# zenlc2000/pycuda-euler

Hardware: AMD Instinct MI355X
Metric: k-mers/sec (encode+hash+deBruijn+Euler), 10Mx100bp k=31, 1/2/4/8 GPU (higher is better)
Workload: dtype u64

## Files before the change

pycuda-euler_amd/csrc/assemble.hip:

```cpp
#include "common.h"
#include "count_global.h"
#include "graph.h"

#include <rocprim/rocprim.hpp>

#include <algorithm>
#include <cmath>
#include <climits>
#include <cstring>
#include <cstddef>
#include <functional>
#include <type_traits>
#include <vector>

#include "count_part.h"
#include "count_v2.h"
#include "count_sk2.h"
#include "shard.h"
#include "compact.h"
#include "count_wide.h"
#include "hostin.h"
#include "join_w.h"
#include "extended.h"
#include "rank_tile.h"
#include "junction.h"
#include "join_local.h"
#include "clip.h"
#include "pop.h"
#include "spectrum.h"
#include "dense_filter.h"

#include <atomic>
#include <chrono>
#include <dlfcn.h>
#include <cstdio>
#include <cstdlib>
#include <mutex>
#include <thread>

namespace ec {

std::atomic<unsigned long long> g_hbm_held{0}, g_hbm_peak{0};
inline void hbm_account(long long d) {
    const unsigned long long now = g_hbm_held.fetch_add((unsigned long long)d) + (unsigned long long)d;
    unsigned long long pk = g_hbm_peak.load();
    while (now > pk && !g_hbm_peak.compare_exchange_weak(pk, now)) {
    }
}
bool memlog_on();

struct DevBuf {
    void *p = nullptr;
    size_t cap = 0;
    __attribute__((noinline)) int ensure(size_t bytes, unsigned int spare_div = 0) {
        if (bytes <= cap) return EC_OK;
        size_t want = std::max<size_t>(bytes, 256);
        if (cap) want += want / 8;
        else if (spare_div) want += want / spare_div;
        release();
        const auto t0 = std::chrono::steady_clock::now();
        if (hipMalloc(&p, want) != hipSuccess) {
            p = nullptr;
            set_error("hipMalloc(%zu) failed", want);
            return EC_ERR_NOMEM;
        }
        cap = want;
        hbm_account((long long)want);
        if (want >= (1ull << 30) && memlog_on()) {
            Dl_info di{};
            void *ra = __builtin_return_address(0);
            const unsigned long off = dladdr(ra, &di) && di.dli_fbase ? (unsigned long)((char *)ra - (char *)di.dli_fbase) : 0ul;
            const double ms = std::chrono::duration<double, std::milli>(std::chrono::steady_clock::now() - t0).count();
            fprintf(stderr, "[eulerhip mem] +%.2f GB (held %.2f GB) in %.1f ms at lib+0x%lx\n", want / 1e9,
                    g_hbm_held.load() / 1e9, ms, off);
        }
        return EC_OK;
    }
    template <typename T>
    T *as() const { return reinterpret_cast<T *>(p); }
    void release() {
        if (p) {
            const auto t0 = std::chrono::steady_clock::now();
            hipFree(p);
            hbm_account(-(long long)cap);
            if (cap >= (1ull << 30) && memlog_on())
                fprintf(stderr, "[eulerhip mem] -%.2f GB (held %.2f GB) in %.1f ms\n", cap / 1e9, g_hbm_held.load() / 1e9,
                        std::chrono::duration<double, std::milli>(std::chrono::steady_clock::now() - t0).count());
        }
        p = nullptr;
        cap = 0;
    }
};

struct HostBuf {
    char *p = nullptr;
    size_t cap = 0, size = 0;
    int resize(size_t bytes) {
        size = bytes;
        if (bytes <= cap) return EC_OK;
        if (p) (void)hipHostFree(p);
        p = nullptr;
        cap = 0;
        size_t want = std::max<size_t>(bytes + bytes / 4, 4096);
        if (hipHostMalloc(reinterpret_cast<void **>(&p), want, hipHostMallocDefault) != hipSuccess) {
            p = nullptr;
            size = 0;
            set_error("hipHostMalloc(%zu) failed", want);
            return EC_ERR_NOMEM;
        }
        cap = want;
        return EC_OK;
    }
    char *data() const { return p; }
    bool empty() const { return size == 0; }
    void release() {
        if (p) (void)hipHostFree(p);
        p = nullptr;
        cap = size = 0;
    }
};

template <typename T>
struct PinnedVec {
    HostBuf b;
    size_t n = 0;
    int resize(size_t count) {
        n = count;
        return b.resize(count * sizeof(T));
    }
    T *data() const { return reinterpret_cast<T *>(b.p); }
    size_t size() const { return n; }
    bool empty() const { return n == 0; }
    T &operator[](size_t i) const { return data()[i]; }
    void release() {
        b.release();
        n = 0;
    }
};

}

using namespace ec;

struct ec_session {
    int device = 0;
    hipStream_t stream = nullptr;
    bool own_stream = false;
    DevBuf h_reads, h_offsets;
    DevBuf hll, scal, table, dkey, dcnt, dfc, dft, upal, outdeg, cand, succ, pred, st0, st1;
    DevBuf rid, rlist, nextR, PK, RK, PL, PM;
    DevBuf hist, ftot, cnt, offs, bstart, tot, recs, recs2, sub;
    DevBuf startOf, skeys, svals, skeys2, svals2, cidxOf, clen, coff, chars, cfirst, clast, headOf, tailOf;
    DevBuf lk, lcnt, tmp, dchars, dcounts;
    bool have = false;
    int k = 0;
    ec_stats stats{};
    HostBuf h_chars;
    bool chars_packed = false;
    uint64_t nchars_host = 0;
    HostBuf bounce;
    struct Pend {
        void *dst;
        size_t off, n;
    };
    std::vector<Pend> pend;
    size_t bused = 0;
    hipEvent_t rd_ev = nullptr;
    hipStream_t ostream = nullptr;
    hipEvent_t oev[4] = {nullptr, nullptr, nullptr, nullptr};
    uint64_t last_nchars = 0;
    DevBuf bmark, rt_tb;
    bool bmark_ok = false;
    uint64_t seg_marks = 0;
    struct SkSpec {
        bool valid = false;
        uint64_t G = 0, cap = 0, nreads = 0, read_base = 0, fcap = 0;
        uint32_t M = 0;
        int k = 0, bbits = 0;
    } skspec;
    struct JlSpec {
        bool valid = false, queued = false;
        int bits = 0, k = 0;
        unsigned int ucap = 0, fcap = 0;
    } jlspec;
    DevBuf jl_frec;
    bool graph_follows = false;
    uint64_t spec_cnt[4] = {0, 0, 0, 0};
    PinnedVec<uint64_t> h_coff;
    PinnedVec<uint64_t> h_loff;
    PinnedVec<int64_t> h_links;
    PinnedVec<uint8_t> h_lc8;
    PinnedVec<uint32_t> h_links32;
    bool links_compact = false;
    HostBuf h_blk;
    bool want_dict = false;
    hipEvent_t ev[2 * EC_NSTAGES] = {};
    hipEvent_t kev[2 * EC_NKERNELS] = {};
    bool kused[EC_NKERNELS] = {};
    bool sused[EC_NSTAGES] = {};
    bool events = false;
    bool timing = false;
    bool stage_timing = false;
    unsigned int n_dense = 0;
    bool dense_ok = false;
    bool stats_ok = false;
    unsigned flags = 0;
    DevBuf ocnt, rbc, mbid, mbid2, midx, midx2, gcur, cwalk, ewalk, lc8;
    bool no_index = false;
    uint64_t shard_base = 0;
    const uint64_t *lc_off = nullptr;
    uint64_t lc_n = 0, lc_L = 0;
    DevBuf bnp;
    DevBuf fcur, bb2;
    DevBuf nrec;
    SolidIndex gidx{};
    SolidIndexW gidxw{};
    bool graph_loaded = false;
    bool placed = false;
    uint64_t seg_lo = 0, seg_Ur = 0;
    DevBuf jrec, joid, jout, jseg, jcnt;
    DevBuf xrec;
    DevBuf skm_rec, skm_ev, skm_end;
    DevBuf wcodes_tab;
    HostBuf hmeta;
    int owner_rule = 0;
    bool own_valid = false;
    int own_rule = 0, own_nowners = 0;
    unsigned int own_n = 0, own_nblk = 0;
    std::vector<unsigned int> own_hi;
    hipStream_t cstream = nullptr;
    struct Pipe {
        bool active = false;
        bool packed = false;
        int nchunks = 0, done = 0;
        std::vector<uint64_t> blo, bhi;
        std::vector<uint64_t> ravail;
        std::vector<uint64_t> elo, ehi;
        uint64_t first_len = 0;
        const uint32_t *codes = nullptr;
        const uint64_t *exc_pos = nullptr;
        const uint8_t *exc_byte = nullptr;
        uint8_t *ascii = nullptr;
        std::vector<hipEvent_t> ev;
    } pipe;
    DevBuf p_codes, p_exc;
    struct Staged {
        Pipe pipe;
        DevBuf codes, exc, off;
        hipEvent_t free_ev = nullptr;
        uint64_t nreads = 0, nbases = 0;
    } stg[2];
    int stg_head = 0, stg_n = 0;
    bool xalpha = false;
    XAlpha xa{};
    DevBuf x_par, x_irr, x_in, x_succ, x_done, x_lk, x_lv, x_lk2, x_lv2, x_len, x_m, x_cid, x_head, x_tail;
    DevBuf jl_kof, jl_rs, jl_re, jl_cnt, jl_off, jl_flag;
    DevBuf rpack;
    DevBuf rt_tcnt, rt_tbase, rt_srec, rt_snrec, rt_sidx, rt_pks, rt_rks, rt_hasp, rt_lr;
    int spec_rounds = 0;
    DevBuf wbv;
    uint64_t seg_n0 = 0, seg_n1 = 0;
    struct Pending {
        int kind = 0;
        uint64_t n = 0;
        unsigned int ntiles = 0;
        bool planned = false;
    } hold;
    SuperRec *chain_scr = nullptr;
    unsigned int seg_nc = 0;
    uint64_t seg_nchars = 0;
    DevBuf run_cnt, run_ends, run_dends;
    DevBuf rt_lb;
    unsigned long long lb_epoch = 0;
    uint64_t run_nr = 0, run_nch = 0, run_nends = 0;
    bool runs_ready = false;
    int part_stage = 0;
    bool clip_ok = false;
    const char *clip_why = "a new session holds no assembly";
    SolidIndex cidx{};
    SolidIndexW cidxw{};
    DevBuf clip_cand, clip_list, clip_kill, clip_tot;
    DevBuf pop_key, pop_sum, pop_tcnt, pop_toff, pop_tile;
    DevBuf spec_hist;
};

static const char *const CLIP_WHY_STEPWISE =
    "the last calls were stepwise ones (ec_count_shard / ec_merge_owned* / ec_graph_*), which leave no one-GPU assembly";

static inline void drop_step_state(ec_session *s) {
    s->hold.kind = 0;
    s->runs_ready = false;
    s->chain_scr = nullptr;
    s->part_stage = 0;
}

namespace {
constexpr size_t BOUNCE_CAP = 64 << 10, BOUNCE_MAX = 16 << 10;

int d2h(ec_session *s, void *dst, const void *src, size_t n, hipStream_t st) {
    if (!n) return EC_OK;
    const size_t off = (s->bused + 15) & ~size_t(15);
    if (n > BOUNCE_MAX || off + n > BOUNCE_CAP) {
        EC_HIP(hipMemcpyAsync(dst, src, n, hipMemcpyDeviceToHost, st));
        return EC_OK;
    }
    if (!s->bounce.p) EC_CHECK(s->bounce.resize(BOUNCE_CAP));
    EC_HIP(hipMemcpyAsync(s->bounce.p + off, src, n, hipMemcpyDeviceToHost, st));
    s->pend.push_back({dst, off, n});
    s->bused = off + n;
    return EC_OK;
}

int host_wait(ec_session *s, hipEvent_t ev) {
    const hipError_t e = hipEventSynchronize(ev);
    for (const auto &q : s->pend) std::memcpy(q.dst, s->bounce.p + q.off, q.n);
    s->pend.clear();
    s->bused = 0;
    if (e != hipSuccess) {
        set_error("HIP error %s", hipGetErrorString(e));
        return EC_ERR_HIP;
    }
    return EC_OK;
}

int host_sync(ec_session *s, hipStream_t st) {
    const hipError_t e = hipStreamSynchronize(st);
    for (const auto &q : s->pend) std::memcpy(q.dst, s->bounce.p + q.off, q.n);
    s->pend.clear();
    s->bused = 0;
    if (e != hipSuccess) {
        set_error("HIP error %s", hipGetErrorString(e));
        return EC_ERR_HIP;
    }
    return EC_OK;
}
}

namespace ec {

template <typename Ops>
__global__ void __launch_bounds__(256) k_kmers_to_agg(const char *chars, const unsigned int *counts, uint64_t n, int k,
                                                      typename RecOf<typename Ops::K>::T *out, unsigned long long *bad) {
    using K = typename Ops::K;
    const K mask = Ops::mask(k);
    for (uint64_t t = blockIdx.x * (uint64_t)blockDim.x + threadIdx.x; t < n; t += (uint64_t)gridDim.x * blockDim.x) {
        const char *x = chars + t * (uint64_t)k;
        K code{};
        bool ok = true;
        for (int i = 0; i < k; i++) {
            const uint32_t b = base_code((unsigned char)x[i]);
            ok &= b < 4;
            code = Ops::push(code, b & 3u, mask);
        }
        if (!ok) atomicMin(bad, (unsigned long long)t);
        const K tw = Ops::twin(code, k);
        out[t] = RecOf<K>::make(code < tw ? code : tw, code <= tw ? counts[t] : 0u,
                                code <= tw ? (unsigned long long)t : ~0ull, tw <= code ? (unsigned long long)t : ~0ull);
    }
}
}

namespace {

struct Scalars {
    unsigned long long npos;
    unsigned long long bad;
    unsigned long long ndistinct;
    double est;
    unsigned int overflow;
    unsigned int nsolid;
    unsigned int nstarts;
    unsigned int final_sel;
    unsigned int ndict;
    unsigned int nr;
    unsigned int npal;
    unsigned int ngath;
    unsigned long long nvisited;
    unsigned int maxlocal;
    unsigned int skew;
    unsigned int lens[4];
    unsigned long long nrec;
    unsigned int nasym, nxl, nxs;
    unsigned int xbad;
    unsigned int wbv_long, wpad;
    unsigned long long chains;
    unsigned int active[64];
};
static_assert(sizeof(Scalars) % 8 == 0 && offsetof(Scalars, bad) % 8 == 0, "k_scal_reset writes 64-bit words");

__global__ void __launch_bounds__(64) k_scal_reset(Scalars *sc) {
    unsigned long long *w = reinterpret_cast<unsigned long long *>(sc);
    for (unsigned int i = threadIdx.x; i < sizeof(Scalars) / 8; i += 64)
        w[i] = i == offsetof(Scalars, bad) / 8 ? ~0ull : 0ull;
}

__global__ void __launch_bounds__(256) k_emit_init(unsigned int *a, unsigned int *b, unsigned int *c, uint64_t n,
                                                   unsigned int *flag) {
    const uint64_t t0 = blockIdx.x * (uint64_t)blockDim.x + threadIdx.x, st = (uint64_t)gridDim.x * blockDim.x;
    if (t0 == 0) *flag = 0;
    const uint64_t n4 = n / 4;
    const uint4 v = make_uint4(0xFFFFFFFFu, 0xFFFFFFFFu, 0xFFFFFFFFu, 0xFFFFFFFFu);
    uint4 *a4 = reinterpret_cast<uint4 *>(a), *b4 = reinterpret_cast<uint4 *>(b), *c4 = reinterpret_cast<uint4 *>(c);
    for (uint64_t i = t0; i < n4; i += st) {
        a4[i] = v;
        b4[i] = v;
        c4[i] = v;
    }
    for (uint64_t i = 4 * n4 + t0; i < n; i += st) a[i] = b[i] = c[i] = 0xFFFFFFFFu;
}

int scan_u64(ec_session *s, const unsigned long long *in, unsigned long long *out, size_t n) {
    size_t bytes = 0;
    EC_HIP(rocprim::exclusive_scan(nullptr, bytes, in, out, 0ull, n, rocprim::plus<unsigned long long>(), s->stream));
    EC_CHECK(s->tmp.ensure(bytes));
    EC_HIP(rocprim::exclusive_scan(s->tmp.p, bytes, in, out, 0ull, n, rocprim::plus<unsigned long long>(), s->stream));
    return EC_OK;
}

int scan_excl_u32(ec_session *s, const unsigned int *in, unsigned int *out, size_t n) {
    size_t bytes = 0;
    EC_HIP(rocprim::exclusive_scan(nullptr, bytes, in, out, 0u, n, rocprim::plus<unsigned int>(), s->stream));
    EC_CHECK(s->tmp.ensure(bytes));
    EC_HIP(rocprim::exclusive_scan(s->tmp.p, bytes, in, out, 0u, n, rocprim::plus<unsigned int>(), s->stream));
    return EC_OK;
}

int scan_incl_u32(ec_session *s, const unsigned int *in, unsigned int *out, size_t n) {
    size_t bytes = 0;
    EC_HIP(rocprim::inclusive_scan(nullptr, bytes, in, out, n, rocprim::plus<unsigned int>(), s->stream));
    EC_CHECK(s->tmp.ensure(bytes));
    EC_HIP(rocprim::inclusive_scan(s->tmp.p, bytes, in, out, n, rocprim::plus<unsigned int>(), s->stream));
    return EC_OK;
}

int sort_pairs(ec_session *s, unsigned long long *kin, unsigned long long *kout, unsigned int *vin, unsigned int *vout,
               size_t n) {
    size_t bytes = 0;
    EC_HIP(rocprim::radix_sort_pairs(nullptr, bytes, kin, kout, vin, vout, n, 0, 64, s->stream));
    EC_CHECK(s->tmp.ensure(bytes));
    EC_HIP(rocprim::radix_sort_pairs(s->tmp.p, bytes, kin, kout, vin, vout, n, 0, 64, s->stream));
    return EC_OK;
}

int pipe_upto(ec_session *s, int c) {
    auto &pp = s->pipe;
    if (!pp.active) return EC_OK;
    c = std::min(c, pp.nchunks - 1);
    if (pp.done > c) return EC_OK;
    const int first = pp.done;
    for (; pp.done <= c; pp.done++) EC_HIP(hipStreamWaitEvent(s->stream, pp.ev[pp.done], 0));
    const uint64_t blo = pp.blo[first], bhi = pp.bhi[c], elo = pp.elo[first], ehi = pp.ehi[c];
    if (pp.packed && bhi > blo) {
        const uint64_t units = ((bhi + 15) >> 4) - (blo >> 4);
        k_unpack2<<<grid_for(units, 256, 16384), 256, 0, s->stream>>>(pp.codes, blo, bhi, pp.ascii);
        if (ehi > elo)
            k_patch<<<grid_for(ehi - elo, 256, 4096), 256, 0, s->stream>>>(pp.exc_pos, pp.exc_byte, elo, ehi,
                                                                           pp.ascii);
    }
    return EC_OK;
}
int pipe_all(ec_session *s) { return s->pipe.active ? pipe_upto(s, s->pipe.nchunks - 1) : EC_OK; }

inline void mark(ec_session *s, int idx) {
    if (s->stage_timing) {
        hipEventRecord(s->ev[idx], s->stream);
        if (idx & 1) s->sused[idx >> 1] = true;
    }
}
inline void kmark(ec_session *s, int kid, int end) {
    if (s->timing) {
        hipEventRecord(s->kev[2 * kid + end], s->stream);
        if (end) s->kused[kid] = true;
    }
}

void collect_timing(ec_session *s) {
    if (!s->timing) return;
    hipStreamSynchronize(s->stream);
    for (int i = 0; i < EC_NSTAGES; i++) {
        float ms = 0;
        if (s->stage_timing && s->sused[i]) hipEventElapsedTime(&ms, s->ev[2 * i], s->ev[2 * i + 1]);
        s->stats.stage_ms[i] = ms;
    }
    for (int i = 0; i < EC_NKERNELS; i++) {
        float ms = 0;
        if (s->kused[i]) hipEventElapsedTime(&ms, s->kev[2 * i], s->kev[2 * i + 1]);
        s->stats.kernel_ms[i] = ms;
    }
}

int begin_call(ec_session *s, int k, unsigned flags) {
    s->xalpha = false;
    drop_step_state(s);
    s->graph_loaded = false;
    s->dense_ok = false;
    s->clip_ok = false;
    s->clip_why = "the session's last call failed";
    refresh_knobs();
    s->have = false;
    s->stats_ok = false;
    if (k < 1 || k > EC_MAX_K) {
        set_error("k=%d outside [1,%d]", k, EC_MAX_K);
        return EC_ERR_ARG;
    }
    EC_HIP(hipSetDevice(s->device));
    if (s->ostream) EC_HIP(hipStreamSynchronize(s->ostream));
    memset(&s->stats, 0, sizeof(s->stats));
    s->k = k;
    s->want_dict = (flags & EC_FLAG_WANT_DICT) != 0;
    s->flags = flags;
    s->shard_base = 0;
    s->own_valid = false;
    s->bmark_ok = false;
    s->seg_marks = 0;
    s->placed = false;
    const bool timing = (flags & (EC_FLAG_TIMING | EC_FLAG_KERNEL_TIMING)) != 0;
    s->stage_timing = (flags & EC_FLAG_TIMING) != 0;
    if (timing && !s->events) {
        for (auto &e : s->ev) EC_HIP(hipEventCreate(&e));
        for (auto &e : s->kev) EC_HIP(hipEventCreate(&e));
        s->events = true;
    }
    s->timing = timing;
    for (auto &u : s->kused) u = false;
    for (auto &u : s->sused) u = false;
    EC_CHECK(s->scal.ensure(sizeof(Scalars)));
    s->jlspec.queued = false;
    s->graph_follows = false;
    k_scal_reset<<<1, 64, 0, s->stream>>>(s->scal.as<Scalars>());
    return EC_OK;
}


template <typename SlotT, typename KeyT>
int compact_table(ec_session *s, SlotT *table, uint64_t cap, long long limit, KeyT *dkey) {
    hipStream_t st = s->stream;
    Scalars *dsc = s->scal.as<Scalars>();
    const unsigned int nblk = (unsigned int)((cap + COMPACT_CHUNK - 1) / COMPACT_CHUNK);
    EC_CHECK(s->rbc.ensure((size_t)nblk * 8 + 8));
    unsigned int *bc = s->rbc.as<unsigned int>(), *bs = bc + nblk;
    EC_HIP(hipMemsetAsync(&dsc->nsolid, 0, 4, st));
    EC_HIP(hipMemsetAsync(&dsc->ndistinct, 0, 8, st));
    k_compact_count<SlotT><<<nblk, 256, 0, st>>>(table, cap, limit, bc, &dsc->ndistinct);
    EC_CHECK(scan_incl_u32(s, bc, bs, nblk));
    k_compact_write<SlotT, KeyT><<<nblk, 256, 0, st>>>(table, cap, limit, bs, dkey, s->dcnt.as<unsigned int>(),
                                                      s->dfc.as<unsigned long long>(),
                                                      s->dft.as<unsigned long long>());
    k_compact_total<<<1, 1, 0, st>>>(bs, nblk, &dsc->nsolid);
    return EC_OK;
}


int check_node_ids(unsigned int U) {
    if (2ull * U >= (unsigned long long)CYC) {
        set_error("too many solid k-mers (%u) for 31-bit node ids", U);
        return EC_ERR_CAPACITY;
    }
    return EC_OK;
}

int check_alphabet(const uint8_t *d_reads, unsigned long long bad) {
    if (bad == ~0ull) return EC_OK;
    uint8_t byte = 0;
    hipMemcpy(&byte, d_reads + bad, 1, hipMemcpyDeviceToHost);
    set_error("byte %llu (0x%02x) outside {A,C,G,T,N}", bad, byte);
    return EC_ERR_ALPHABET;
}

struct BucketArgs {
    const unsigned long long *bbeg = nullptr, *bend = nullptr;
    bool filt = false;
    int pmin = 0, pmax = 1;
    unsigned int *bmark = nullptr;
};
BucketArgs filter_args(bool filt, int pmax) {
    BucketArgs a;
    a.filt = filt;
    a.pmax = pmax;
    a.pmin = kn().filter_pmin >= 0 ? std::max(0, std::min(pmax, kn().filter_pmin)) : 0;
    return a;
}

template <typename Src>
int launch_bucket(ec_session *s, Src src, unsigned nb, unsigned slots, long long limit, BucketArgs a = {}) {
    Scalars *dsc = s->scal.as<Scalars>();
    hipStream_t st = s->stream;
    const unsigned long long *bb = a.bbeg ? a.bbeg : s->bstart.as<unsigned long long>();
    const unsigned long long *be = a.bbeg ? a.bend : s->bstart.as<unsigned long long>() + 1;
    if (a.filt) {
        EC_CHECK(s->bnp.ensure(nb));
        k_bucket_filt<Src><<<nb, BUCKET_THREADS, 0, st>>>(
            src, bb, be, 1u, limit, a.pmin, a.pmax, (float)PART_KEYS,
            s->dkey.as<unsigned long long>(),
            s->dcnt.as<unsigned int>(), s->dfc.as<unsigned long long>(), s->dft.as<unsigned long long>(),
            s->no_index ? nullptr : s->sub.as<SubSlot>(), s->bnp.as<uint8_t>(), &dsc->nsolid, &dsc->ndistinct,
            &dsc->overflow);
        return EC_OK;
    }
    if (slots == 2048)
        k_bucket<Src, 2048><<<nb, BUCKET_THREADS, 0, st>>>(
            src, bb, be, 1u, limit, s->dkey.as<unsigned long long>(), s->dcnt.as<unsigned int>(),
            s->dfc.as<unsigned long long>(), s->dft.as<unsigned long long>(), s->no_index ? nullptr : s->sub.as<SubSlot>(), &dsc->nsolid,
            &dsc->ndistinct, &dsc->overflow, a.bmark);
    else
        k_bucket<Src, 4096><<<nb, BUCKET_THREADS, 0, st>>>(
            src, bb, be, 1u, limit, s->dkey.as<unsigned long long>(), s->dcnt.as<unsigned int>(),
            s->dfc.as<unsigned long long>(), s->dft.as<unsigned long long>(), s->no_index ? nullptr : s->sub.as<SubSlot>(), &dsc->nsolid,
            &dsc->ndistinct, &dsc->overflow, a.bmark);
    return EC_OK;
}

struct BucketPlan {
    bool part = false;
    bool filt = false;
    int pmax = 1;
    int bbits = 0;
    unsigned int slots = 2048;
};
BucketPlan plan_buckets(double est, long long limit) {
    constexpr int PMAX = 3;
    BucketPlan p;
    const double filt_max = limit >= 1 ? 32768.0 : PART_KEYS * (1 << PMAX);
    p.part = est / FINE <= 2400.0 || est / FINE <= filt_max;
    p.filt = p.part && (est / FINE > 2400.0 || kn().force_filter);
    while (p.pmax < PMAX && est / FINE / (double)(1 << p.pmax) > PART_KEYS) p.pmax++;
    if (kn().filter_pmax) p.pmax = std::max(1, std::min(PMAX, kn().filter_pmax));
    while (p.bbits < FINE_BITS && est / (double)(1ull << p.bbits) > 1100.0) p.bbits++;
    p.slots = p.filt ? (2048u << p.pmax) : est / (double)(1ull << p.bbits) > 1100.0 ? 4096u : 2048u;
    return p;
}

static uint64_t skpart_slots(int npf, int w, bool val) {
    static thread_local int cache[3][SK_W_MAX + 1][2] = {};
    const int ni = npf == 4 ? 0 : npf == 7 ? 1 : 2;
    int &c = cache[ni][w][val];
    if (!c) {
        const void *fn = nullptr;
#define EC_SKF(NPF, W)                                                                                        \
    if (npf == NPF && w == W) fn = val ? (const void *)&k_skpart_w<NPF, W, true> : (const void *)&k_skpart_w<NPF, W, false>;
#define EC_SKF_W(W) EC_SKF(4, W) EC_SKF(7, W) EC_SKF(10, W)
        EC_SKF_W(7) EC_SKF_W(8) EC_SKF_W(9) EC_SKF_W(10) EC_SKF_W(11) EC_SKF_W(12)
        EC_SKF_W(13) EC_SKF_W(14) EC_SKF_W(15) EC_SKF_W(16) EC_SKF_W(17) EC_SKF_W(18)
#undef EC_SKF_W
#undef EC_SKF
        int dev = 0, ncu = 0, per = 0;
        if (!fn || hipGetDevice(&dev) != hipSuccess ||
            hipDeviceGetAttribute(&ncu, hipDeviceAttributeMultiprocessorCount, dev) != hipSuccess ||
            hipOccupancyMaxActiveBlocksPerMultiprocessor(&per, fn, PT_THREADS, 0) != hipSuccess || per < 1)
            return 1;
        c = ncu * per;
    }
    return (uint64_t)c;
}

int phase_count_sk2(ec_session *s, const uint8_t *d_reads, const uint64_t *d_off, uint64_t nreads,
                    uint64_t read_base, int k, long long limit, uint32_t M, uint64_t G, uint64_t gsize, uint64_t P,
                    int npf, unsigned int &U, SolidIndex &sidx, bool &done, bool validate = false,
                    bool *invalid = nullptr) {
    done = false;
    if (invalid) *invalid = false;
    if (k >= SK_MIN_K && k <= 32) {
        const uint64_t ntiles = (nreads + 63) / 64, slots = skpart_slots(npf, k - SK_M + 1, validate);
        uint64_t g = std::max<uint64_t>(1, std::min<uint64_t>(ntiles, RF_MAX_RUNS));
        if (g > slots) g = g / slots * slots;
        gsize = ((ntiles + g - 1) / g) * 64;
        G = (nreads + gsize - 1) / gsize;
    }
    if (k < SK_MIN_K || k > 32 || M > 256 || gsize * M >= (1ull << 24) || (read_base + nreads) * 2 * M >= (1ull << 32) ||
        kn().no_sk2)
        return EC_OK;
    hipStream_t st = s->stream;
    Scalars *dsc = s->scal.as<Scalars>();
    Scalars hsc;
    auto reset = [&]() -> int {
        if (validate) {
            EC_HIP(hipMemsetAsync(dsc, 0, sizeof(Scalars), st));
            EC_HIP(hipMemsetAsync(&dsc->bad, 0xFF, sizeof(unsigned long long), st));
            return EC_OK;
        }
        EC_HIP(hipMemsetAsync(&dsc->overflow, 0, sizeof(unsigned int), st));
        EC_HIP(hipMemsetAsync(&dsc->skew, 0, sizeof(unsigned int), st));
        EC_HIP(hipMemsetAsync(&dsc->nsolid, 0, sizeof(unsigned int), st));
        EC_HIP(hipMemsetAsync(&dsc->ndistinct, 0, sizeof(unsigned long long), st));
        return EC_OK;
    };
    const MinCfg mc = sk_cfg(k);
    constexpr uint64_t C = 1ull << SK2_CBITS;
    const double per_read = 2.0 * M / (mc.w + 1) + 2.0;
    const uint64_t cap = (uint64_t)(gsize * per_read * 1.4 / C) + 256;
    EC_CHECK(s->recs.ensure((C * G * cap + SK2_ECAP_W) * 16));
    EC_CHECK(s->cnt.ensure(C * G * 4));
    EC_CHECK(s->hll.ensure(G * (1 << HLL_REG_BITS)));
    EC_CHECK(s->ftot.ensure((1 << HLL_REG_BITS) * 4));
    uint4 *recs = s->recs.as<uint4>();
    const uint32_t smask = P >= (1ull << 26) ? 255u : 0u;
    unsigned int *hreg = s->ftot.as<unsigned int>();
    if (!validate) EC_HIP(hipMemsetAsync(&dsc->nrec, 0, sizeof(unsigned long long), st));
    mark(s, 2 * EC_STAGE_COUNT);
    kmark(s, 1, 0);
#define EC_SKPART_WV(NPF, W, VAL)                                                                             \
    k_skpart_w<NPF, W, VAL><<<lgb - lga, PT_THREADS, 0, st>>>(                                                   \
        d_reads, d_off, nreads, mc, M, gsize, (uint32_t)G, cap, smask, recs, s->cnt.as<unsigned int>(),          \
        s->hll.as<uint8_t>(), &dsc->nrec, &dsc->overflow, &dsc->lens[2], &dsc->npos, lga, elim)
#define EC_SKPART_W(NPF, W)            \
    if (validate)                      \
        EC_SKPART_WV(NPF, W, true);    \
    else                               \
        EC_SKPART_WV(NPF, W, false)
#define EC_SKPART_NPF(W)              \
    if (npf == 4) EC_SKPART_W(4, W);  \
    else if (npf == 7) EC_SKPART_W(7, W); \
    else EC_SKPART_W(10, W)
    const bool chunked = s->pipe.active && s->pipe.done < s->pipe.nchunks;
    if (!chunked) EC_CHECK(pipe_all(s));
    unsigned lga = 0, lgb = (unsigned)G;
    const uint32_t elim = kn().sk2_elim >= 128 ? (uint32_t)std::min(kn().sk2_elim, SK2_ECAP_W) : (uint32_t)SK2_ECAP_W;
    for (int pc = chunked ? 0 : s->pipe.nchunks; ; pc++) {
      if (chunked) {
        if (pc >= s->pipe.nchunks) break;
        lgb = pc + 1 == s->pipe.nchunks ? (unsigned)G : (unsigned)std::min<uint64_t>(G, s->pipe.ravail[pc] / gsize);
        if (lgb <= lga) continue;
        EC_CHECK(pipe_upto(s, pc));
      }
      {
        switch (mc.w) {
            case 7: EC_SKPART_NPF(7); break;
            case 8: EC_SKPART_NPF(8); break;
            case 9: EC_SKPART_NPF(9); break;
            case 10: EC_SKPART_NPF(10); break;
            case 11: EC_SKPART_NPF(11); break;
            case 12: EC_SKPART_NPF(12); break;
            case 13: EC_SKPART_NPF(13); break;
            case 14: EC_SKPART_NPF(14); break;
            case 15: EC_SKPART_NPF(15); break;
            case 16: EC_SKPART_NPF(16); break;
            case 17: EC_SKPART_NPF(17); break;
            default: EC_SKPART_NPF(18); break;
        }
      }
      if (!chunked) break;
      lga = lgb;
    }
#undef EC_SKPART_NPF
#undef EC_SKPART_W
#undef EC_SKPART_WV
    kmark(s, 1, 1);
    EC_HIP(hipMemsetAsync(hreg, 0, (1 << HLL_REG_BITS) * 4, st));
    k_hll_merge<<<dim3((1 << HLL_REG_BITS) / 256, TOT_SLICES), 256, 0, st>>>(s->hll.as<uint8_t>(), G, hreg);
    k_hll_final<<<1, 1024, 0, st>>>(hreg, HLL_REG_BITS, &dsc->est);
    EC_CHECK(d2h(s, &hsc, dsc, sizeof(Scalars), st));
    auto launch_refine = [&](int bb, uint64_t fc) -> int {
        const uint64_t nb = 1ull << bb;
        EC_CHECK(s->recs2.ensure(nb * fc * 16));
        EC_CHECK(s->fcur.ensure(nb * 8));
        EC_CHECK(s->bb2.ensure(nb * 16));
        EC_HIP(hipMemsetAsync(s->fcur.p, 0, nb * 8, st));
        unsigned rs = 8;
        if (kn().refine_rs) rs = (unsigned)std::max(1, kn().refine_rs);
        rs = (unsigned)std::min<uint64_t>(rs, G);
        kmark(s, 4, 0);
        k_skrefine<<<dim3((unsigned)C, rs), BUCKET_THREADS, 0, st>>>(recs, s->cnt.as<unsigned int>(), (uint32_t)G, cap,
                                                                      bb, s->recs2.as<uint4>(), fc,
                                                                      s->fcur.as<unsigned long long>(), &dsc->skew, M,
                                                                      gsize, read_base, k);
        kmark(s, 4, 1);
        unsigned long long *b0 = s->bb2.as<unsigned long long>();
        k_fixed_bounds<<<grid_for(nb, 256), 256, 0, st>>>(s->fcur.as<unsigned long long>(), nb, fc, b0, b0 + nb);
        return EC_OK;
    };
    const auto sp = s->skspec;
    const bool spec = sp.valid && sp.G == G && sp.cap == cap && sp.nreads == nreads && sp.read_base == read_base &&
                      sp.M == M && sp.k == k && !chunked && kn().no_spec == 0;
    s->skspec.valid = false;
    if (spec) {
        if (!s->rd_ev) EC_HIP(hipEventCreateWithFlags(&s->rd_ev, hipEventDisableTiming));
        EC_HIP(hipEventRecord(s->rd_ev, st));
        EC_CHECK(launch_refine(sp.bbits, sp.fcap));
        EC_CHECK(host_wait(s, s->rd_ev));
    } else {
        EC_CHECK(host_sync(s, st));
    }
    const bool verbose = kn().verbose;
    if (validate) {
        if (hsc.lens[2]) {
            if (verbose) fprintf(stderr, "count_sk2: input needs the prescan\n");
            if (invalid) *invalid = true;
            return reset();
        }
        P = hsc.npos;
    }
    if (hsc.overflow) {
        if (verbose) fprintf(stderr, "count_sk2: partition run overflow (cap %llu)\n", (unsigned long long)cap);
        return reset();
    }
    const double est = hsc.est * (smask + 1.0);
    BucketPlan plan = plan_buckets(est, limit);
    const bool skfilt = plan.part && plan.filt && limit >= 1 && kn().sk_filt != 0 &&
                        est / (double)(1ull << SK2_BBITS) <= 16000.0;
    if (!plan.part || (plan.filt && !skfilt)) return reset();
    int bbits = SK2_CBITS;
    const bool b3 = !skfilt && !kn().no_skb3 && est / (double)(1ull << SK2_BBITS) <= 380.0;
    const double per_bucket = b3 ? 380.0 : 800.0;
    while (bbits < SK2_BBITS && est / (double)(1ull << bbits) > per_bucket) bbits++;
    if (skfilt) bbits = SK2_BBITS;
    plan.bbits = bbits;
    plan.slots = skfilt ? 2048u : b3 ? 1024u : est / (double)(1ull << bbits) > 1100.0 ? 4096u : 2048u;
    const uint64_t Bk = 1ull << bbits;
    const uint64_t NR = hsc.nrec;
    uint64_t fcap = NR * 2 / Bk + 1024;
    const bool refine_stood = spec && sp.bbits == bbits && sp.fcap >= fcap && sp.fcap <= fcap + fcap / 8;
    if (refine_stood) {
        fcap = sp.fcap;
    } else {
        if (spec && verbose) fprintf(stderr, "count_sk2: refine plan changed (bits %d -> %d), refined again\n", sp.bbits, bbits);
        fcap += fcap / 16;
        EC_CHECK(launch_refine(bbits, fcap));
    }
    s->skspec.valid = true;
    s->skspec.G = G;
    s->skspec.cap = cap;
    s->skspec.nreads = nreads;
    s->skspec.read_base = read_base;
    s->skspec.fcap = fcap;
    s->skspec.M = M;
    s->skspec.k = k;
    s->skspec.bbits = bbits;
    unsigned long long *bbeg = s->bb2.as<unsigned long long>(), *bend = bbeg + Bk;
    mark(s, 2 * EC_STAGE_COUNT + 1);

    mark(s, 2 * EC_STAGE_COMPACT);
    const uint64_t umax = Bk * plan.slots;
    EC_CHECK(s->dkey.ensure(umax * 8));
    EC_CHECK(s->dcnt.ensure(umax * 4));
    EC_CHECK(s->dfc.ensure(umax * 8));
    EC_CHECK(s->dft.ensure(umax * 8));
    EC_CHECK(s->sub.ensure(umax * sizeof(SubSlot)));
    bool b3_marked = false;
    for (int attempt = 0;; attempt++) {
    kmark(s, 2, 0);
    const double inv_m = 1.0 / M;
#define EC_SKBUCKET_ARGS                                                                                     \
    s->recs2.as<uint4>(), bbeg, bend, k, M, inv_m, limit, s->dkey.as<unsigned long long>(),                    \
        s->dcnt.as<unsigned int>(), s->dfc.as<unsigned long long>(), s->dft.as<unsigned long long>(),          \
        s->no_index ? nullptr : s->sub.as<SubSlot>(), &dsc->nsolid, &dsc->ndistinct, &dsc->overflow
#define EC_SKBUCKET(SLOTS, RS, EVEN) \
    k_skbucket<SLOTS, RS, 1, EVEN><<<(unsigned)Bk, BUCKET_THREADS, 0, st>>>(EC_SKBUCKET_ARGS, dbg)
    b3_marked = false;
    unsigned long long *dbg = nullptr;
    if (kn().sk2_stats) {
        EC_CHECK(s->tmp.ensure(128));
        dbg = s->tmp.as<unsigned long long>();
        EC_HIP(hipMemsetAsync(dbg, 0, 128, st));
    }
    if (skfilt) {
        constexpr int NTF = 512;
        const unsigned int max_keys = kn().skf_keys > 0 ? (unsigned int)kn().skf_keys : 1900u;
        unsigned int *bm = nullptr;
        if (kn().skf_merge != 0) {
            EC_CHECK(s->skm_rec.ensure(Bk * fcap * sizeof(uint4)));
            EC_CHECK(s->skm_ev.ensure(Bk * fcap * sizeof(uint2)));
            EC_CHECK(s->skm_end.ensure(Bk * 8));
            uint4 *mrec = s->skm_rec.as<uint4>();
            uint2 *mev = s->skm_ev.as<uint2>();
            unsigned long long *mend = s->skm_end.as<unsigned long long>();
            const unsigned int claim_cap = kn().sk2_claim > 0 ? (unsigned int)kn().sk2_claim : ~0u;
            if (kn().skf_merge != 2)
                k_skdedup<4096, 1024><<<(unsigned)Bk, 1024, 0, st>>>(s->recs2.as<uint4>(), bbeg, bend, k, M, inv_m, mrec,
                                                                     mev, mend, claim_cap, dbg);
            else
                k_skdedup<2560, 512><<<(unsigned)Bk, 512, 0, st>>>(s->recs2.as<uint4>(), bbeg, bend, k, M, inv_m, mrec,
                                                                   mev, mend, claim_cap, dbg);
#define EC_SKF_MERGED_ARGS                                                                                   \
    mrec, bbeg, mend, k, M, inv_m, limit, s->dkey.as<unsigned long long>(), s->dcnt.as<unsigned int>(),      \
        s->dfc.as<unsigned long long>(), s->dft.as<unsigned long long>(),                                    \
        s->no_index ? nullptr : s->sub.as<SubSlot>(), &dsc->nsolid, &dsc->ndistinct, &dsc->overflow, max_keys, \
        dbg, bm, mev
            if (k & 1)
                k_skbucket_filt<2048, NTF, false, true><<<(unsigned)Bk, NTF, 0, st>>>(EC_SKF_MERGED_ARGS);
            else
                k_skbucket_filt<2048, NTF, true, true><<<(unsigned)Bk, NTF, 0, st>>>(EC_SKF_MERGED_ARGS);
#undef EC_SKF_MERGED_ARGS
        } else if (k & 1)
            k_skbucket_filt<2048, NTF, false><<<(unsigned)Bk, NTF, 0, st>>>(EC_SKBUCKET_ARGS, max_keys, dbg, bm);
        else
            k_skbucket_filt<2048, NTF, true><<<(unsigned)Bk, NTF, 0, st>>>(EC_SKBUCKET_ARGS, max_keys, dbg, bm);
        b3_marked = bm != nullptr;
    } else if (plan.slots == 1024) {
        constexpr int NT3 = 512;
        const unsigned int claim_cap = kn().sk2_claim > 0 ? (unsigned int)kn().sk2_claim : ~0u;
        const size_t words = (umax / 32 + 2 + 63) & ~size_t(63);
        EC_CHECK(s->bmark.ensure(words * 4));
        EC_HIP(hipMemsetAsync(s->bmark.p, 0, words * 4, st));
        unsigned int *bm = s->bmark.as<unsigned int>();
        if (dbg) {
            if (k & 1)
                k_skbucket3<1024, 1664, NT3, false, true><<<(unsigned)Bk, NT3, 0, st>>>(EC_SKBUCKET_ARGS, dbg, claim_cap, bm);
            else
                k_skbucket3<1024, 1664, NT3, true, true><<<(unsigned)Bk, NT3, 0, st>>>(EC_SKBUCKET_ARGS, dbg, claim_cap, bm);
        } else if (k & 1)
            k_skbucket3<1024, 1664, NT3, false><<<(unsigned)Bk, NT3, 0, st>>>(EC_SKBUCKET_ARGS, dbg, claim_cap, bm);
        else
            k_skbucket3<1024, 1664, NT3, true><<<(unsigned)Bk, NT3, 0, st>>>(EC_SKBUCKET_ARGS, dbg, claim_cap, bm);
        b3_marked = true;
    } else if (plan.slots == 2048) {
        if (k & 1) EC_SKBUCKET(2048, 3072, false);
        else EC_SKBUCKET(2048, 3072, true);
    } else {
        if (k & 1) EC_SKBUCKET(4096, 2048, false);
        else EC_SKBUCKET(4096, 2048, true);
    }
#undef EC_SKBUCKET
#undef EC_SKBUCKET_ARGS
    if (dbg) {
        unsigned long long h[16];
        EC_CHECK(d2h(s, h, dbg, 128, st));
        EC_CHECK(host_sync(s, st));
        const double nw = (double)Bk * ((plan.slots == 1024 ? 512 : BUCKET_THREADS) / 64);
        if (skfilt)
            fprintf(stderr, "k_skbucket_filt: %llu buckets: max distinct est %llu, max predicted inserts %llu, max "
                            "seen-twice cells %llu, max records %llu; refused by the predictor %llu, tables filled "
                            "%llu, most keys inserted %llu; most merged records %llu, most past the claim cap %llu, "
                            "merged records %llu of %llu\n",
                    (unsigned long long)Bk, h[0], h[1], h[2], h[3], h[4], h[5], h[6], h[7], h[8], h[9],
                    (unsigned long long)NR);
        if (plan.slots == 1024)
            fprintf(stderr, "k_skbucket3: %llu buckets, most distinct records in a bucket %llu\n",
                    (unsigned long long)Bk, h[3]);
        fprintf(stderr, "k_skbucket per wave (shader clocks): records phase canon %.0f probe %.0f (%.1f iterations) "
                        "post %.0f barrier %.0f over %.1f rounds; roll-out %.0f barrier %.0f\n",
                h[8] / nw, h[9] / nw, h[11] / nw, h[10] / nw, h[12] / nw, h[13] / nw, h[14] / nw, h[15] / nw);
        fprintf(stderr, "k_skbucket: %llu records, %llu distinct in %llu flushes (%.2f / bucket), %llu windows rolled "
                        "(positions %llu); block-us: init %.0f records %.0f sort %.0f roll-out %.0f finish %.0f\n",
                (unsigned long long)NR, h[0], h[1], (double)h[1] / Bk, h[2], (unsigned long long)P, h[3] / 100.0,
                h[4] / 100.0, h[5] / 100.0, h[6] / 100.0, h[7] / 100.0);
    }
    kmark(s, 2, 1);
    mark(s, 2 * EC_STAGE_COMPACT + 1);
    EC_CHECK(d2h(s, &hsc, dsc, sizeof(Scalars), st));
    const auto jp = s->jlspec;
    s->jlspec.queued = false;
    if (!attempt && refine_stood && jp.valid && s->graph_follows && !s->no_index && !skfilt && !dbg &&
        (k & 1) && jp.k == k && jp.bits == bbits && kn().jl_bits_delta == 0 && kn().jl_fcap <= 0 &&
        kn().join_links != 0 && kn().join_local != 0) {
        const unsigned int ntab = 1u << jp.bits;
        EC_CHECK(s->jl_kof.ensure((size_t)jp.ucap * 4));
        EC_CHECK(s->jl_rs.ensure((size_t)ntab * 4));
        EC_CHECK(s->jl_re.ensure((size_t)ntab * 4));
        EC_CHECK(s->jl_cnt.ensure(((size_t)ntab + 1) * 4));
        EC_CHECK(s->jl_off.ensure(((size_t)ntab + 1) * 4));
        EC_CHECK(s->jl_flag.ensure((size_t)(JL_NCTR + 1) * JL_CSTRIDE * 4));
        EC_CHECK(s->jl_frec.ensure((size_t)jp.fcap * sizeof(RecJ64)));
        EC_CHECK(s->upal.ensure(jp.ucap));
        EC_CHECK(s->succ.ensure((size_t)jp.ucap * 8));
        if (!s->rd_ev) EC_HIP(hipEventCreateWithFlags(&s->rd_ev, hipEventDisableTiming));
        EC_HIP(hipEventRecord(s->rd_ev, st));
        unsigned int *flags = s->jl_flag.as<unsigned int>();
        k_jl_init<<<grid_for(2ull * jp.ucap, 256, 4096), 256, 0, st>>>(
            flags, (JL_NCTR + 1) * JL_CSTRIDE, s->jl_rs.as<unsigned int>(), s->jl_cnt.as<unsigned int>(), ntab,
            s->succ.as<unsigned int>(), 2ull * jp.ucap, s->upal.as<uint8_t>(), jp.ucap);
        k_jl_scan<unsigned long long><<<grid_for(jp.ucap, 256, 8192), 256, 0, st>>>(
            s->dkey.as<unsigned long long>(), jp.ucap, k, jp.bits, s->upal.as<uint8_t>(), s->jl_kof.as<unsigned int>(),
            s->jl_frec.as<RecJ64>(), flags + JL_CSTRIDE, jp.fcap, s->jl_cnt.as<unsigned int>(),
            s->jl_rs.as<unsigned int>(), s->jl_re.as<unsigned int>(), &flags[1], &dsc->nsolid, &flags[2]);
        EC_CHECK(host_wait(s, s->rd_ev));
        s->jlspec.queued = true;
        if (hsc.skew || hsc.overflow || hsc.nsolid > jp.ucap) {
            s->jlspec.queued = false;
            s->spec_cnt[1]++;
        }
    } else {
        EC_CHECK(host_sync(s, st));
    }
    if (!hsc.skew || attempt) break;
    std::vector<unsigned long long> hcur(Bk);
    EC_CHECK(d2h(s, hcur.data(), s->fcur.p, Bk * 8, st));
    EC_CHECK(host_sync(s, st));
    const uint64_t need = *std::max_element(hcur.begin(), hcur.end());
    if (need <= fcap || need > 4 * fcap || Bk * need * 16 > (1ull << 30)) break;
    if (verbose)
        fprintf(stderr, "count_sk2: final bucket overflow (fcap %llu), refined again with capacity %llu\n",
                (unsigned long long)fcap, (unsigned long long)need);
    fcap = need;
    EC_HIP(hipMemsetAsync(&dsc->overflow, 0, sizeof(unsigned int), st));
    EC_HIP(hipMemsetAsync(&dsc->skew, 0, sizeof(unsigned int), st));
    EC_HIP(hipMemsetAsync(&dsc->nsolid, 0, sizeof(unsigned int), st));
    EC_HIP(hipMemsetAsync(&dsc->ndistinct, 0, sizeof(unsigned long long), st));
    EC_CHECK(launch_refine(bbits, fcap));
    }
    if (hsc.overflow || hsc.skew) {
        if (verbose)
            fprintf(stderr, "count_sk2: %s overflow (%llu buckets, %u slots, est %.0f, fcap %llu)\n",
                    hsc.skew ? "final bucket" : "table", (unsigned long long)Bk, plan.slots, est,
                    (unsigned long long)fcap);
        s->stats.table_retries++;
        return reset();
    }
    done = true;
    s->bmark_ok = b3_marked;
    s->stats.n_positions = P;
    s->stats.n_distinct_est = (uint64_t)llround(est);
    s->stats.record_bytes = 16;
    s->stats.n_records = NR;
    s->stats.count_path = EC_PATH_PARTITIONED;
    s->stats.count_variant = 3;
    s->stats.n_buckets = (uint32_t)Bk;
    s->stats.table_capacity = umax;
    sidx = SolidIndex{};
    sidx.sub = s->sub.as<SubSlot>();
    sidx.bbits = bbits;
    sidx.slots = plan.slots;
    sidx.sk = 1;
    sidx.mc = mc;
    sidx.npb = nullptr;
    U = hsc.nsolid;
    s->stats.n_distinct = hsc.ndistinct;
    s->stats.n_solid = U;
    return check_node_ids(U);
}

int phase_count_v2(ec_session *s, const uint8_t *d_reads, const uint64_t *d_off, uint64_t nreads, uint64_t read_base,
                   int k, long long limit, bool allow_sk2, unsigned int &U, SolidIndex &sidx, bool &ok) {
    ok = false;
    hipStream_t st = s->stream;
    Scalars *dsc = s->scal.as<Scalars>();
    Scalars hsc;
    const uint64_t ntiles = (nreads + 63) / 64;
    uint64_t gmax = RF_MAX_RUNS;
    uint64_t G = std::max<uint64_t>(1, std::min<uint64_t>(ntiles, gmax));
    const uint64_t gsize = ((ntiles + G - 1) / G) * 64;
    G = (nreads + gsize - 1) / gsize;
    auto npf_of = [](uint64_t lall) {
        const uint64_t need16 = (64ull * lall + 30 + 15) / 16;
        return need16 <= 4 * 64 ? 4 : need16 <= 7 * 64 ? 7 : need16 <= 10 * 64 ? 10 : 0;
    };
    if (allow_sk2 && k >= SK_MIN_K && k <= 32 && !kn().no_sk2) {
        uint64_t L = s->lc_L;
        if (s->pipe.active) {
            L = s->pipe.first_len;
        } else if (!(L >= (uint64_t)k && npf_of(L) && s->lc_off == d_off && s->lc_n == nreads)) {
            uint64_t o2[2] = {0, 0};
            EC_CHECK(d2h(s, o2, d_off, 16, st));
            EC_CHECK(host_sync(s, st));
            L = o2[1] - o2[0];
        }
        s->lc_L = 0;
        const int npf = npf_of(L);
        if (L >= (uint64_t)k && npf) {
            const uint32_t M = (uint32_t)(L - k + 1);
            bool done = false, invalid = false;
            mark(s, 2 * EC_STAGE_PRESCAN);
            mark(s, 2 * EC_STAGE_PRESCAN + 1);
            EC_CHECK(phase_count_sk2(s, d_reads, d_off, nreads, read_base, k, limit, M, G, gsize, nreads * M, npf, U,
                                     sidx, done, true, &invalid));
            if (done) {
                if (!s->pipe.active) s->lc_off = d_off, s->lc_n = nreads, s->lc_L = L;
                ok = true;
                return EC_OK;
            }
            if (!invalid) allow_sk2 = false;
        }
    }
    EC_CHECK(pipe_all(s));
    mark(s, 2 * EC_STAGE_PRESCAN);
    kmark(s, 0, 0);
    k_prescan<<<(unsigned)G, 256, 0, st>>>(d_reads, d_off, nreads, k, gsize, &dsc->npos, &dsc->bad, dsc->lens);
    kmark(s, 0, 1);
    mark(s, 2 * EC_STAGE_PRESCAN + 1);
    EC_CHECK(d2h(s, &hsc, dsc, sizeof(Scalars), st));
    EC_CHECK(host_sync(s, st));
    EC_CHECK(check_alphabet(d_reads, hsc.bad));
    const unsigned int lmax = hsc.lens[0], lmin = ~hsc.lens[1], lall = hsc.lens[3];
    const uint64_t P = hsc.npos;
    if (hsc.lens[2] || P == 0 || lmax != lmin) return EC_OK;
    const uint32_t M = lmax - (uint32_t)k + 1;
    int ibits = 1;
    while ((1ull << ibits) < M) ibits++;
    if (ibits > 15 || nreads + read_base > (1ull << (31 - ibits)) || 2ull * M - 1 > MAX_LOCAL_EVENT) return EC_OK;
    const int npf = npf_of(lall);
    if (!npf) return EC_OK;
    if (allow_sk2) {
        bool done = false;
        EC_CHECK(phase_count_sk2(s, d_reads, d_off, nreads, read_base, k, limit, M, G, gsize, P, npf, U, sidx, done));
        if (done) {
            ok = true;
            return EC_OK;
        }
    }

    auto nbits = [](uint64_t x) {
        int b = 0;
        while ((1ull << b) < x) b++;
        return b;
    };
    const int r10env = kn().v2_r10;
    const bool r10 = r10env != 0 && (r10env == 1 || P >= (1ull << 26)) && k >= 16 &&
                     (2 * k - PT_CBITS) + std::max(0, nbits(gsize) + 1 + ibits - 16) <= 64;

    constexpr uint64_t C = 1ull << PT_CBITS;
    const uint64_t cap = (gsize * M * 5 / 4 + C - 1) / C + 128;
    EC_CHECK(s->recs.ensure((C * G * cap + PT_REC) * 12));
    EC_CHECK(s->cnt.ensure(C * G * 4));
    EC_CHECK(s->hll.ensure(G * (1 << HLL_REG_BITS)));
    EC_CHECK(s->ftot.ensure((1 << HLL_REG_BITS) * 4));
    unsigned long long *rkeys = s->recs.as<unsigned long long>();
    unsigned int *rmeta = reinterpret_cast<unsigned int *>(rkeys + C * G * cap + PT_REC);
    const uint32_t smask = P >= (1ull << 26) ? 255u : 0u;
    unsigned int *hreg = s->ftot.as<unsigned int>();
    mark(s, 2 * EC_STAGE_COUNT);
    kmark(s, 1, 0);
#define EC_PARTITION(NPF, HI, R10)                                                                            \
    k_partition<NPF, HI, R10><<<(unsigned)G, PT_THREADS, 0, st>>>(d_reads, d_off, nreads, k, M, gsize, (uint32_t)G, \
                                                                   cap, ibits, read_base, smask, rkeys, rmeta,        \
                                                                   s->cnt.as<unsigned int>(),                         \
                                                                   s->hll.as<uint8_t>(), &dsc->overflow)
#define EC_PARTITION_R(NPF, HI)        \
    if (r10)                           \
        EC_PARTITION(NPF, HI, true);   \
    else                               \
        EC_PARTITION(NPF, HI, false)
    if (k >= 17) {
        if (npf == 4) EC_PARTITION_R(4, true);
        else if (npf == 7) EC_PARTITION_R(7, true);
        else EC_PARTITION_R(10, true);
    } else {
        if (npf == 4) EC_PARTITION_R(4, false);
        else if (npf == 7) EC_PARTITION_R(7, false);
        else EC_PARTITION_R(10, false);
    }
#undef EC_PARTITION_R
#undef EC_PARTITION
    kmark(s, 1, 1);
    EC_HIP(hipMemsetAsync(hreg, 0, (1 << HLL_REG_BITS) * 4, st));
    k_hll_merge<<<dim3((1 << HLL_REG_BITS) / 256, TOT_SLICES), 256, 0, st>>>(s->hll.as<uint8_t>(), G, hreg);
    k_hll_final<<<1, 1024, 0, st>>>(hreg, HLL_REG_BITS, &dsc->est);
    EC_CHECK(d2h(s, &hsc, dsc, sizeof(Scalars), st));
    EC_CHECK(host_sync(s, st));
    if (hsc.overflow) return EC_OK;
    const double est = hsc.est * (smask + 1.0);
    BucketPlan plan = plan_buckets(est, limit);
    if (!plan.part) return EC_OK;
    plan.bbits = std::max(plan.bbits, PT_CBITS);
    const int bbits = plan.bbits;
    const uint64_t Bk = 1ull << bbits;

    const uint64_t fcap = P * 5 / 4 / Bk + 1024;
    EC_CHECK(s->recs2.ensure(Bk * fcap * 12));
    EC_CHECK(s->fcur.ensure(Bk * 8));
    EC_CHECK(s->bb2.ensure(Bk * 16));
    EC_HIP(hipMemsetAsync(s->fcur.p, 0, Bk * 8, st));
    unsigned rs = 8;
    if (kn().refine_rs) rs = (unsigned)std::max(1, kn().refine_rs);
    rs = (unsigned)std::min<uint64_t>(rs, G);
    kmark(s, 4, 0);
#define EC_REFINE(IN10)                                                                                           \
    k_refine2<IN10><<<dim3((unsigned)C, rs), BUCKET_THREADS, 0, st>>>(                                          \
        rkeys, rmeta, s->cnt.as<unsigned int>(), (uint32_t)G, cap, bbits, s->recs2.as<unsigned int>(), fcap,     \
        s->fcur.as<unsigned long long>(), &dsc->skew, k, ibits, gsize, read_base)
    if (r10)
        EC_REFINE(true);
    else
        EC_REFINE(false);
#undef EC_REFINE
    kmark(s, 4, 1);
    unsigned long long *bbeg = s->bb2.as<unsigned long long>(), *bend = bbeg + Bk;
    k_fixed_bounds<<<grid_for(Bk, 256), 256, 0, st>>>(s->fcur.as<unsigned long long>(), Bk, fcap, bbeg, bend);
    mark(s, 2 * EC_STAGE_COUNT + 1);

    mark(s, 2 * EC_STAGE_COMPACT);
    const uint64_t umax = Bk * plan.slots;
    EC_CHECK(s->dkey.ensure(umax * 8));
    EC_CHECK(s->dcnt.ensure(umax * 4));
    EC_CHECK(s->dfc.ensure(umax * 8));
    EC_CHECK(s->dft.ensure(umax * 8));
    EC_CHECK(s->sub.ensure(umax * sizeof(SubSlot)));
    BucketArgs ba = filter_args(plan.filt, plan.pmax);
    ba.bbeg = bbeg;
// ... 4180 lines not shown
```

pycuda-euler_amd/csrc/capi.cpp:

```cpp
#include <cstdarg>
#include <cstdio>
#include <cstdlib>

#include "common.h"

namespace ec {
static thread_local char g_err[512] = "";

void set_error(const char *fmt, ...) {
    va_list ap;
    va_start(ap, fmt);
    vsnprintf(g_err, sizeof g_err, fmt, ap);
    va_end(ap);
}

static thread_local Knobs g_knobs;
const Knobs &kn() { return g_knobs; }
void refresh_knobs() {
    Knobs k;
    if (getenv("EULERHIP_DEBUG")) {
        auto flag = [](const char *n) { return getenv(n) != nullptr; };
        auto num = [](const char *n, int dflt) {
            const char *e = getenv(n);
            return e ? atoi(e) : dflt;
        };
        k.no_sk2 = flag("EULERHIP_NO_SK2");
        k.force_filter = flag("EULERHIP_FORCE_FILTER");
        k.filter_pmax = num("EULERHIP_FILTER_PMAX", 0);
        k.filter_pmin = num("EULERHIP_FILTER_PMIN", -1);
        k.v2_r10 = num("EULERHIP_V2_R10", -1);
        k.refine_rs = num("EULERHIP_REFINE_RS", 0);
        k.no_spec = num("EULERHIP_NO_SPEC", 0);
        k.rank_sync = num("EULERHIP_RANK_SYNC", 0);
        k.skf_merge = num("EULERHIP_SKF_MERGE", 1);
        k.wide_runs = num("EULERHIP_WIDE_RUNS", 1);
        k.no_small_starts = flag("EULERHIP_NO_SMALL_STARTS");
        k.wide_max_bbits = num("EULERHIP_WIDE_MAX_BBITS", -1);
        k.wide_l3 = num("EULERHIP_WIDE_L3", 0);
        k.join_links = num("EULERHIP_JOIN_LINKS", -1);
        k.join_cap = num("EULERHIP_JOIN_CAP", 0);
        k.junction_bt = num("EULERHIP_JUNCTION_BT", -1);
        k.sk2_elim = num("EULERHIP_SK2_ELIM", 0);
        k.no_char_pack = num("EULERHIP_NO_CHAR_PACK", 0);
        k.junction_sb = num("EULERHIP_JUNCTION_SB", 0);
        k.junction_claim = num("EULERHIP_JUNCTION_CLAIM", 0);
        if (const char *e = getenv("EULERHIP_WIDE_L3_CAP")) k.wide_l3_cap = atoll(e);
        k.host_chunks = num("EULERHIP_HOST_CHUNKS", 0);
        k.sk2_stats = flag("EULERHIP_SK2_STATS");
        k.no_skb3 = flag("EULERHIP_NO_SKB3");
        k.sk2_claim = num("EULERHIP_SK2_CLAIM", 0);
        k.verbose = flag("EULERHIP_VERBOSE");
        k.rank = num("EULERHIP_RANK", -1);
        k.sk_filt = num("EULERHIP_SK_FILT", -1);
        k.skf_keys = num("EULERHIP_SKF_KEYS", 0);
        k.wide_mb = num("EULERHIP_WIDE_MB", -1);
        k.join_mb = num("EULERHIP_JOIN_MB", -1);
        k.join_local = num("EULERHIP_JOIN_LOCAL", -1);
        k.junction_radix = num("EULERHIP_JUNCTION_RADIX", -1);
        k.jl_fcap = num("EULERHIP_JL_FCAP", -1);
        k.jl_bits_delta = num("EULERHIP_JL_BITS_DELTA", 0);
    }
    g_knobs = k;
}
bool memlog_on() {
    static const bool on = getenv("EULERHIP_MEMLOG") != nullptr;
    return on;
}
}

extern "C" const char *ec_last_error(void) { return ec::g_err; }
extern "C" int ec_version(void) { return 500;  }

extern "C" int ec_spectrum_threshold(const uint64_t *h, uint32_t nbins, ec_spectrum_info *info) {
    if (nbins < 2 || nbins > EC_SPECTRUM_MAX_BINS) {
        ec::set_error("ec_spectrum_threshold: nbins %u outside [2, %d]", nbins, EC_SPECTRUM_MAX_BINS);
        return EC_ERR_ARG;
    }
    if (!h || !info) {
        ec::set_error("ec_spectrum_threshold: null hist / info");
        return EC_ERR_ARG;
    }
    *info = ec_spectrum_info{};
    uint32_t lo = 0;
    while (lo < nbins && !h[lo]) lo++;
    if (lo == nbins) return EC_OK;
    info->lo = lo;
    uint32_t d = lo;
    while (d + 1 < nbins && h[d] >= h[d + 1]) d++;
    if (d + 1 >= nbins) return EC_OK;
    info->descent_end = d;
    if (d == lo) return EC_OK;
    uint32_t p = d;
    for (uint32_t c = d + 1; c < nbins; c++)
        if (h[c] > h[p]) p = c;
    info->peak = p;
    if (p == nbins - 1) return EC_OK;
    uint64_t m = h[lo];
    for (uint32_t c = lo; c <= p; c++) m = h[c] < m ? h[c] : m;
    info->floor = m;
    uint32_t v = lo;
    const uint64_t within = (h[p] - m) / EC_SPECTRUM_FLOOR_DIV;
    while (v < p && h[v] - m > within) v++;
    if (v == p) return EC_OK;
    info->found = 1;
    info->limit = v;
    return EC_OK;
}
```

pycuda-euler_amd/csrc/common.h:

```cpp
#pragma once
#include <cstring>
#include <hip/hip_runtime.h>
#include <stdint.h>
#include <stdio.h>
#include <string>

#include "../../include/eulerhip.h"

namespace ec {

constexpr uint32_t NONE32 = 0xFFFFFFFFu;
constexpr uint64_t NONE64 = ~0ull;
constexpr uint64_t EMPTY_KEY = ~0ull;

void set_error(const char *fmt, ...);

struct Knobs {
    bool no_sk2 = false;
    bool force_filter = false;
    int filter_pmax = 0;
    int filter_pmin = -1;
    int v2_r10 = -1;
    int refine_rs = 0;
    int rank_sync = 0;
    int no_spec = 0;
    int skf_merge = 1;
    int wide_runs = 1;
    int wide_max_bbits = -1;
    int wide_l3 = 0;
    long long wide_l3_cap = 0;
    int wide_mb = -1;
    int join_links = -1;
    int join_cap = 0;
    int join_local = -1;
    int join_mb = -1;
    int jl_fcap = -1;
    int jl_bits_delta = 0;
    int junction_bt = -1;
    int junction_sb = 0;
    int junction_claim = 0;
    int junction_radix = -1;
    int no_char_pack = 0;
    int sk2_elim = 0;
    int sk2_claim = 0;
    bool sk2_stats = false;
    bool no_skb3 = false;
    int sk_filt = -1;
    int skf_keys = 0;
    int host_chunks = 0;
    bool verbose = false;
    int rank = -1;
    bool no_small_starts = false;
};
void refresh_knobs();
const Knobs &kn();

#define EC_HIP(call)                                                                       \
    do {                                                                                   \
        hipError_t e_ = (call);                                                            \
        if (e_ != hipSuccess) {                                                            \
            ::ec::set_error("%s:%d %s -> %s", __FILE__, __LINE__, #call, hipGetErrorString(e_)); \
            return EC_ERR_HIP;                                                             \
        }                                                                                  \
    } while (0)

#define EC_CHECK(call)                 \
    do {                               \
        int rc_ = (call);              \
        if (rc_ != EC_OK) return rc_;  \
    } while (0)

__host__ __device__ inline uint64_t kmask64(int k) { return k >= 32 ? ~0ull : ((1ull << (2 * k)) - 1); }

__host__ __device__ inline uint64_t rev2_64(uint64_t x) {
    x = ((x >> 2) & 0x3333333333333333ull) | ((x & 0x3333333333333333ull) << 2);
    x = ((x >> 4) & 0x0F0F0F0F0F0F0F0Full) | ((x & 0x0F0F0F0F0F0F0F0Full) << 4);
#if defined(__HIP_DEVICE_COMPILE__)
    return __builtin_bswap64(x);
#else
    return __builtin_bswap64(x);
#endif
}

__host__ __device__ inline uint64_t twin64(uint64_t x, int k) { return rev2_64(x ^ kmask64(k)) >> (64 - 2 * k); }

__host__ __device__ inline uint64_t mix64(uint64_t x) {
    x ^= x >> 29;
    x *= 0xbf58476d1ce4e5b9ull;
    x ^= x >> 32;
    return x;
}

constexpr uint64_t BIJ_C = 0xbf58476d1ce4e5b9ull;
constexpr uint64_t BIJ_CINV = 0x96de1b173f119089ull;
__host__ __device__ inline uint64_t bij_fwd(uint64_t x, int s, uint64_t m) {
    x ^= x >> s;
    x = (x * BIJ_C) & m;
    return x ^ (x >> s);
}
__host__ __device__ inline uint64_t bij_inv(uint64_t x, int s, uint64_t m) {
    x ^= x >> s;
    x = (x * BIJ_CINV) & m;
    return x ^ (x >> s);
}

__device__ inline uint32_t base_code(uint32_t c) {
    switch (c) {
    case 'A': return 0;
    case 'C': return 1;
    case 'G': return 2;
    case 'T': return 3;
    case 'N': return 4;
    default: return 5;
    }
}

__device__ inline unsigned int wave_append(unsigned int *counter, bool pred) {
    const unsigned long long m = __ballot(pred);
    if (!m) return 0;
    const unsigned int lane = threadIdx.x & 63;
    const int leader = __ffsll((long long)m) - 1;
    unsigned int base = 0;
    if ((int)lane == leader) base = atomicAdd(counter, (unsigned int)__popcll(m));
    base = __shfl(base, leader);
    return base + (unsigned int)__popcll(m & ((1ull << lane) - 1));
}

inline unsigned grid_for(uint64_t n, unsigned block, unsigned cap = 1u << 20) {
    uint64_t g = (n + block - 1) / block;
    if (g < 1) g = 1;
    if (g > cap) g = cap;
    return (unsigned)g;
}

}
```

pycuda-euler_amd/csrc/count_sk2.h:

```cpp
#pragma once
#include "count_v2.h"
#include "superkmer.h"

namespace ec {

constexpr int SK2_NMAX = 16;
constexpr int SK2_ECAP_W = 1024;
constexpr int SK2_FLUSH_AT = SK2_ECAP_W - 64 - 640;
#ifndef SK2_PD_DEF
#define SK2_PD_DEF 4
#endif
constexpr int SK2_PD = SK2_PD_DEF;
constexpr int SK2_HQ = 128;
constexpr int SK2_BASES = 46;
#ifndef SK2_TILE_DEF
#define SK2_TILE_DEF 2048
#endif
constexpr int SK2_TILE = SK2_TILE_DEF;
constexpr int SK2_CBITS = 6;
constexpr int SK2_BBITS = 14;
constexpr int SK2_FBITS = SK2_BBITS - SK2_CBITS;

__host__ __device__ constexpr inline uint32_t sk2_nmax(int k) {
    return (uint32_t)(SK2_BASES - k + 1 < SK2_NMAX ? SK2_BASES - k + 1 : SK2_NMAX);
}

__device__ inline uint32_t sk_bases16(const uint32_t *st, uint32_t p) {
    return __builtin_amdgcn_alignbit(st[(p >> 4) + 1], st[p >> 4], 2 * (p & 15));
}
__device__ inline void sk_hll_put(unsigned int *s_hll, uint32_t hh) {
    const uint32_t hj = hh >> (32 - HLL_REG_BITS);
    const uint32_t rho = (uint32_t)__clz((int)((hh << HLL_REG_BITS) | (1u << (HLL_REG_BITS - 1)))) + 1;
    const uint32_t hs = (hj & 3) * 8;
    uint32_t old = s_hll[hj >> 2];
    while (rho > ((old >> hs) & 0xFFu)) {
        const uint32_t nw = (old & ~(0xFFu << hs)) | (rho << hs);
        const uint32_t prev = atomicCAS(&s_hll[hj >> 2], old, nw);
        if (prev == old) break;
        old = prev;
    }
}

template <int C>
__device__ inline void skpart_flush(uint32_t cntw, const uint32_t *ent, uint16_t *srt, unsigned int *wcnt,
                                    unsigned int *cur, unsigned long long *base, const uint32_t *rel,
                                    const uint32_t *st, uint32_t lane, unsigned long long gcap, uint64_t cap,
                                    unsigned long long spill, uint32_t M, uint32_t rtile, uint4 *recs,
                                    unsigned int *overflow, unsigned int *s_hll, uint32_t *hq, uint32_t smaskb,
                                    int k, uint64_t kmask) {
    wave_sync();
    for (uint32_t i = lane; i < cntw; i += 64) atomicAdd(&wcnt[ent[i] >> 26], 1u);
    wave_sync();
    const unsigned int v = lane < (uint32_t)C ? wcnt[lane] : 0u;
    const unsigned int incl = wave_incl_scan(v);
    const unsigned int beg = incl - v;
    if (lane < (uint32_t)C) {
        wcnt[lane] = beg;
        unsigned int at = 0;
        if (v) at = atomicAdd(&cur[lane], v);
        unsigned long long b0 = gcap + lane * cap + at - beg;
        if (at + v > cap) {
            atomicOr(overflow, 1u);
            b0 = spill - beg;
        }
        base[lane] = b0;
    }
    wave_sync();
    for (uint32_t i = lane; i < cntw; i += 64) {
        const unsigned int p = atomicAdd(&wcnt[ent[i] >> 26], 1u);
        srt[p] = (uint16_t)i;
    }
    wave_sync();
    uint32_t nq = 0;
    auto hll_drain = [&]() {
        wave_sync();
        for (uint32_t x = lane; x < nq * SK2_NMAX; x += 64) {
            const uint32_t qe = hq[x / SK2_NMAX], q = x % SK2_NMAX;
            if (q <= (qe >> 16)) {
                const uint32_t p = (qe & 0xFFFFu) + q;
                const uint64_t K = (uint64_t)sk_bases16(st, p) | (uint64_t)sk_bases16(st, p + 16) << 32;
                const uint64_t krc = ~K & kmask, kfw = rev2_64(K) >> (64 - 2 * k);
                sk_hll_put(s_hll, (uint32_t)(mix64(kfw < krc ? kfw : krc) >> 32));
            }
        }
        wave_sync();
        nq = 0;
    };
    for (uint32_t i0 = 0; i0 < cntw; i0 += 64) {
        const uint32_t i = i0 + lane;
        bool samp = false;
        uint32_t qv = 0;
        if (i < cntw) {
            const uint32_t e = ent[srt[i]];
            const uint32_t lr = e & 63u, w0 = (e >> 6) & 0xFFu, n1 = (e >> 14) & 15u;
            const uint32_t p0 = rel[lr] + w0;
            uint4 o;
            o.x = sk_bases16(st, p0);
            o.y = sk_bases16(st, p0 + 16);
            o.z = (sk_bases16(st, p0 + 32) & 0x0FFFFFFFu) | n1 << 28;
            o.w = ((e >> 18) & ((1u << SK2_FBITS) - 1)) << 24 | ((rtile + lr) * M + w0);
            recs[base[e >> 26] + i] = o;
            samp = ((e >> 18) & smaskb) == 0;
            qv = p0 | n1 << 16;
        }
        const uint64_t sb = __builtin_amdgcn_ballot_w64(samp);
        if (samp) hq[nq + __builtin_amdgcn_mbcnt_hi((uint32_t)(sb >> 32), __builtin_amdgcn_mbcnt_lo((uint32_t)sb, 0u))] = qv;
        nq += (uint32_t)__popcll(sb);
        if (nq > (uint32_t)(SK2_HQ - 64)) hll_drain();
    }
    if (nq) hll_drain();
    wave_sync();
    if (lane < (uint32_t)C) wcnt[lane] = 0;
}

template <int NPF, int W, bool VAL>
__global__ void __launch_bounds__(PT_THREADS) k_skpart_w(const uint8_t *__restrict__ buf,
                                                         const uint64_t *__restrict__ off, uint64_t nreads, MinCfg mc,
                                                         uint32_t M, uint64_t gsize, uint32_t G, uint64_t cap,
                                                         uint32_t smask, uint4 *recs, unsigned int *cnt, uint8_t *hll,
                                                         unsigned long long *nrec, unsigned int *overflow,
                                                         unsigned int *vfail, unsigned long long *npos,
                                                         uint32_t g_lo, uint32_t elim) {
    constexpr int C = 1 << SK2_CBITS;
    constexpr int NREG = 1 << HLL_REG_BITS;
    constexpr int SW = NPF * 64 + 4;
    static_assert(SK2_FLUSH_AT >= 64, "the entry buffer holds a flush's worth");
    __shared__ uint32_t s_stage[PT_WAVES][SW];
    __shared__ uint32_t s_ent[PT_WAVES][SK2_ECAP_W];
    __shared__ uint16_t s_srt[PT_WAVES][SK2_ECAP_W];
    __shared__ uint32_t s_rel[PT_WAVES][64];
    __shared__ unsigned long long s_base[PT_WAVES][C];
    __shared__ unsigned int s_wcnt[PT_WAVES][C];
    __shared__ unsigned int s_cur[C];
    __shared__ unsigned int s_hll[NREG / 4];
    __shared__ uint32_t s_hq[PT_WAVES][SK2_HQ];
    const uint32_t lane = threadIdx.x & 63;
    const uint32_t wid = __builtin_amdgcn_readfirstlane(threadIdx.x >> 6);
    for (int i = threadIdx.x; i < NREG / 4; i += PT_THREADS) s_hll[i] = 0;
    if (threadIdx.x < C) s_cur[threadIdx.x] = 0;
    if (lane < C) s_wcnt[wid][lane] = 0;
    __syncthreads();
    const uint64_t g = blockIdx.x + (uint64_t)g_lo;
    const uint64_t g0 = min(g * gsize, nreads), g1 = min(g0 + gsize, nreads);
    const uint32_t ntile = (uint32_t)((g1 - g0 + 63) / 64);
    const int k = mc.k;
    constexpr uint32_t nmax = sk2_nmax(W + SK_M - 1);
    const uint64_t kmask = kmask64(k);
    uint4 pf[NPF];
    uint64_t nx_base = 0;
    uint32_t nx_s = 0, nx_e = 0, nx_n = 0, nx_lo = 0, nx_hi = 0, nx_n16 = 0;
    uint32_t nwin = 0;
    if (wid < ntile) EC_PT_ISSUE(wid);
    const unsigned long long gcap = g * C * cap, spill = (unsigned long long)C * G * cap;
    uint32_t *st = s_stage[wid];
    uint32_t *ent = s_ent[wid];
    for (uint32_t t = wid; t < ntile; t += PT_WAVES) {
        if (VAL) {
            uint32_t diff = 0;
#pragma unroll
            for (int q = 0; q < NPF; q++) {
                const uint32_t wv[4] = {pf[q].x, pf[q].y, pf[q].z, pf[q].w};
                uint32_t packed = 0, d[4];
#pragma unroll
                for (int u = 0; u < 4; u++) {
                    const uint32_t x = ((wv[u] >> 1) ^ (wv[u] >> 2)) & 0x03030303u;
                    const uint32_t y = x | (x >> 6);
                    packed |= ((y | (y >> 12)) & 0xFFu) << (8 * u);
                    d[u] = __builtin_amdgcn_perm(0u, 0x54474341u, x) ^ wv[u];
                }
                st[q * 64 + lane] = packed;
                const uint32_t lo = 16 * (q * 64 + lane);
                if (lo >= nx_lo && lo + 16 <= nx_hi) {
                    diff |= d[0] | d[1] | d[2] | d[3];
                } else if (lo < nx_hi && lo + 16 > nx_lo) {
                    const uint32_t from = (uint32_t)min(max((int)nx_lo - (int)lo, 0), 16);
                    const uint32_t to = (uint32_t)min(max((int)nx_hi - (int)lo, 0), 16);
                    const uint32_t m16 = (0xFFFFu >> (16 - to)) & ~((1u << from) - 1u);
#pragma unroll
                    for (int u = 0; u < 4; u++) {
                        const uint32_t m4 = (m16 >> (4 * u)) & 15u;
                        const uint32_t keep = ((m4 * 0x00204081u) & 0x01010101u) * 0xFFu;
                        diff |= d[u] & keep;
                    }
                }
            }
            bool bad = nx_n16 > (uint32_t)NPF * 64 || diff != 0;
            if (lane < nx_n) {
                const uint32_t ln = nx_e - nx_s;
                bad |= ln >= (uint32_t)k && ln != M + (uint32_t)k - 1;
            }
            if (__any(bad) && lane == 0) atomicOr(vfail, 1u);
            nwin += (uint32_t)__popcll(__ballot(lane < nx_n && nx_e - nx_s >= (uint32_t)k));
        } else {
#pragma unroll
            for (int q = 0; q < NPF; q++) st[q * 64 + lane] = pack16(pf[q]);
        }
        const uint32_t tbase = (uint32_t)nx_base, s = nx_s;
        const uint32_t len = lane < nx_n ? nx_e - nx_s : 0u;
        const bool more = t + PT_WAVES < ntile;
        const bool has = len >= (uint32_t)k;
        const uint32_t rel = has ? s - tbase : 0u;
        s_rel[wid][lane] = rel;
        wave_sync();
        constexpr int m = SK_M;
        constexpr uint32_t MMASK = (1u << (2 * SK_M)) - 1;
        uint32_t mf = 0, mr = 0;
        auto push_base = [&](uint32_t b) {
            mf = ((mf << 2) | b) & MMASK;
            mr = (mr >> 2) | ((3u - b) << (2 * SK_M - 2));
        };
        uint32_t S[W];
        {
            const uint32_t x0 = sk_bases16(st, rel), x1 = sk_bases16(st, rel + 16);
#pragma unroll
            for (int tb = 0; tb < m - 1; tb++) push_base(tb < 16 ? (x0 >> (2 * tb)) & 3u : (x1 >> (2 * (tb - 16))) & 3u);
#pragma unroll
            for (int j = 0; j < W; j++) {
                const int tb = m - 1 + j;
                push_base(tb < 16 ? (x0 >> (2 * tb)) & 3u : (x1 >> (2 * (tb - 16))) & 3u);
                S[j] = mmer_hash(mf < mr ? mf : mr);
            }
#pragma unroll
            for (int j = W - 2; j >= 0; j--) S[j] = min(S[j], S[j + 1]);
        }
        const uint32_t nrounds = __any(has) ? (M + W - 1) / W : 0u;
        uint32_t runv = S[0], rsx = 0, cntw = 0;
        const uint64_t hasm = __builtin_amdgcn_ballot_w64(has);
        const uint32_t rtile = 64 * t;
        auto entry = [&](uint32_t end) { return (runv << 18) + lane + (((end - 1u) << 14) + rsx); };
        auto rs_term = [](uint32_t w) { return (uint32_t)((int)w * -16320); };
        for (uint32_t round = 0; round < nrounds; round++) {
            const uint32_t w0 = round * W;
            const uint32_t q = rel + w0 + W;
            const uint32_t a0 = sk_bases16(st, q), a1 = sk_bases16(st, q + 16);
            const uint32_t rw0 = rs_term(w0);
            uint32_t H[W];
            uint32_t P = 0xFFFFFFFFu;
            auto window = [&](int j) {
                const uint32_t v = min(S[j], P);
                const int tb = m - 1 + j;
                const uint32_t b = tb < 16 ? (a0 >> (2 * tb)) & 3u : (a1 >> (2 * (tb - 16))) & 3u;
                mf = (mf << 2) | b;
                const uint32_t fw = mf & MMASK;
                const uint32_t le = j == 0 ? a0 : j < 16 ? __builtin_amdgcn_alignbit(a1, a0, 2 * j) : a1 >> (2 * (j - 16));
                const uint32_t rc = ~le & MMASK;
                H[j] = mmer_hash(fw < rc ? fw : rc);
                P = min(P, H[j]);
                const uint32_t end = w0 + j;
                const bool c1 = v != runv, c2 = rsx == rw0 + (uint32_t)((j - (int)nmax) * -16320);
                const bool close = has & (c1 | c2);
                const uint64_t bal = (__builtin_amdgcn_ballot_w64(c1) | __builtin_amdgcn_ballot_w64(c2)) & hasm;
                if (close) {
                    const uint32_t rk = __builtin_amdgcn_mbcnt_hi((uint32_t)(bal >> 32),
                                                                  __builtin_amdgcn_mbcnt_lo((uint32_t)bal, 0u));
                    ent[min(cntw, elim - 64) + rk] = entry(end);
                    rsx = rw0 + (uint32_t)(j * -16320);
                }
                cntw += (uint32_t)__popcll(bal);
                runv = v;
            };
            if (w0 + W <= M) {
#pragma unroll
                for (int j = 0; j < W; j++) window(j);
            } else {
#pragma unroll
                for (int j = 0; j < W; j++) {
                    if (w0 + j >= M) break;
                    window(j);
                }
            }
#pragma unroll
            for (int j = 0; j < W; j++) S[j] = H[j];
#pragma unroll
            for (int j = W - 2; j >= 0; j--) S[j] = min(S[j], S[j + 1]);
            if (cntw > elim - 64) {
                if (lane == 0) atomicOr(overflow, 1u);
                cntw = elim - 64;
            }
            if (round + 1 < nrounds && cntw > elim - 64 - 640) {
                skpart_flush<C>(cntw, ent, s_srt[wid], s_wcnt[wid], s_cur, s_base[wid], s_rel[wid], st, lane, gcap,
                                cap, spill, M, rtile, recs, overflow, s_hll, s_hq[wid], smask ? 0xFFu : 0u, k,
                                kmask);
                cntw = 0;
            }
        }
        EC_PT_ISSUE(more ? t + PT_WAVES : t);
        if (nrounds) {
            const uint64_t bal = hasm;
            if (has) {
                const uint32_t rk = __builtin_amdgcn_mbcnt_hi((uint32_t)(bal >> 32),
                                                              __builtin_amdgcn_mbcnt_lo((uint32_t)bal, 0u));
                ent[cntw + rk] = entry(M);
            }
            cntw += (uint32_t)__popcll(bal);
            skpart_flush<C>(cntw, ent, s_srt[wid], s_wcnt[wid], s_cur, s_base[wid], s_rel[wid], st, lane, gcap,
                            cap, spill, M, rtile, recs, overflow, s_hll, s_hq[wid], smask ? 0xFFu : 0u, k, kmask);
        }
    }
    __shared__ unsigned int s_nwin[PT_WAVES];
    if (VAL && lane == 0) s_nwin[wid] = nwin;
    __syncthreads();
    if (threadIdx.x < C) cnt[(uint64_t)threadIdx.x * G + g] = (unsigned int)min((uint64_t)s_cur[threadIdx.x], cap);
    if (threadIdx.x == 0) {
        unsigned long long tot = 0;
        for (int c = 0; c < C; c++) tot += s_cur[c];
        if (tot) atomicAdd(nrec, tot);
        if (VAL) {
            unsigned long long wn = 0;
            for (int q = 0; q < PT_WAVES; q++) wn += s_nwin[q];
            if (wn) atomicAdd(npos, wn * M);
        }
    }
    unsigned int *hw = reinterpret_cast<unsigned int *>(hll + g * NREG);
    for (int i = threadIdx.x; i < NREG / 4; i += PT_THREADS) hw[i] = s_hll[i];
}

__device__ inline uint32_t rev2_32b(uint32_t v) {
    v = __builtin_bitreverse32(v);
    return ((v >> 1) & 0x55555555u) | ((v & 0x55555555u) << 1);
}
__device__ inline bool sk2_canon(uint32_t &r0, uint32_t &r1, uint32_t &r2, int k) {
    const unsigned int n = (r2 >> 28) + 1, L2 = 2 * (n + (unsigned int)k - 1);
    const uint32_t m1 = L2 >= 64 ? 0xFFFFFFFFu : (1u << ((L2 - 32) & 31)) - 1u;
    const uint32_t mw2 = L2 > 64 ? (1u << ((L2 - 64) & 31)) - 1u : 0u;
    const uint32_t x0 = r0, x1 = r1 & m1, x2 = r2 & mw2;
    const uint32_t y0 = rev2_32b(x2), y1 = rev2_32b(x1), y2 = rev2_32b(x0);
    const unsigned int sft = 96 - L2, s5 = sft & 31;
    const bool lo = sft < 32;
    const uint32_t a0 = __builtin_amdgcn_alignbit(y1, y0, s5), a1 = __builtin_amdgcn_alignbit(y2, y1, s5),
                   a2 = y2 >> s5;
    const uint32_t q0 = ~(lo ? a0 : a1), q1 = ~(lo ? a1 : a2) & m1, q2 = lo ? ~a2 & mw2 : 0u;
    const bool flip = q2 != x2 ? q2 < x2 : q1 != x1 ? q1 < x1 : q0 < x0;
    r0 = flip ? q0 : x0, r1 = flip ? q1 : x1, r2 = (flip ? q2 : x2) | (n - 1) << 28;
    return flip;
}
__device__ inline void sk2_events(uint32_t w, unsigned int n, uint32_t M, double inv_m, uint32_t &EA, uint32_t &EB) {
    const unsigned int p = w & 0x7FFFFFFFu;
    const bool flip = (w >> 31) != 0;
    const unsigned int rd0 = (unsigned int)((double)p * inv_m);
    int rm = (int)(p - rd0 * M);
    unsigned int rd = rd0;
    if (rm < 0) rd--, rm += (int)M;
    else if (rm >= (int)M) rd++, rm -= (int)M;
    const unsigned int A = rd * 2 * M + (unsigned int)rm, B = rd * 2 * M + 2 * M - 1 - (unsigned int)rm;
    EA = flip ? B - n + 1 : A, EB = flip ? A + n - 1 : B;
}

__global__ void __launch_bounds__(BUCKET_THREADS) k_skrefine(const uint4 *recs, const unsigned int *cnt, uint32_t G,
                                                             uint64_t cap, int bbits, uint4 *out, uint64_t fcap,
                                                             unsigned long long *fcur, unsigned int *overflow,
                                                             uint32_t M, uint64_t gsize, uint64_t read_base, int k) {
    constexpr int TILE = SK2_TILE;
    constexpr int PER = TILE / BUCKET_THREADS;
    constexpr uint64_t C = 1 << SK2_CBITS;
    __shared__ uint4 tile[TILE];
    __shared__ uint8_t tj[TILE];
    __shared__ unsigned long long base[REFINE_FANOUT];
    __shared__ unsigned int tcnt[REFINE_FANOUT], tbeg[REFINE_FANOUT], wsum[BUCKET_THREADS / 64];
    __shared__ unsigned int lst[RF_MAX_RUNS + 1];
    const int fb = bbits - SK2_CBITS;
    const int F = 1 << fb;
    const uint64_t c = blockIdx.x;
    const uint32_t ga = (uint32_t)((uint64_t)G * blockIdx.y / gridDim.y),
                   gb = (uint32_t)((uint64_t)G * (blockIdx.y + 1) / gridDim.y);
    const uint32_t nr = gb - ga;
    const int lane = threadIdx.x & 63, wid = threadIdx.x >> 6;
    {
        const uint32_t i0 = 2 * threadIdx.x;
        const unsigned int a = i0 < nr ? cnt[c * G + ga + i0] : 0u, b = i0 + 1 < nr ? cnt[c * G + ga + i0 + 1] : 0u;
        unsigned int incl = a + b;
        for (int o = 1; o < 64; o <<= 1) {
            const unsigned int u = __shfl_up(incl, o);
            if (lane >= o) incl += u;
        }
        if (lane == 63) wsum[wid] = incl;
        __syncthreads();
        unsigned int before = 0;
        for (int q = 0; q < wid; q++) before += wsum[q];
        const unsigned int ex = before + incl - (a + b);
        if (i0 <= nr) lst[i0] = ex;
        if (i0 + 1 <= nr) lst[i0 + 1] = ex + a;
        __syncthreads();
    }
    const uint64_t N = lst[nr];
    uint32_t j0 = 0;
    for (uint64_t t0 = 0; t0 < N; t0 += TILE) {
        while (j0 + 1 < nr && lst[j0 + 1] <= t0) j0++;
        const unsigned int n = (unsigned int)min((uint64_t)TILE, N - t0);
        if (threadIdx.x < REFINE_FANOUT) tcnt[threadIdx.x] = 0;
        __syncthreads();
        unsigned int rx[PER], ry[PER], rz[PER], rw[PER], lr[PER], jj[PER], rk[PER];
#pragma unroll
        for (int q = 0; q < PER; q++) {
            const unsigned int i = threadIdx.x + q * BUCKET_THREADS;
            if (i < n) {
                const uint64_t l = t0 + i;
                uint32_t jr = j0;
                while (lst[jr + 1] <= l) jr++;
                const uint4 v = recs[((ga + jr) * C + c) * cap + (l - lst[jr])];
                rx[q] = v.x, ry[q] = v.y, rz[q] = v.z, rw[q] = v.w;
                lr[q] = jr;
            }
        }
#pragma unroll
        for (int q = 0; q < PER; q++) {
            const unsigned int i = threadIdx.x + q * BUCKET_THREADS;
            if (i < n) {
                jj[q] = fb ? (rw[q] >> 24) >> (SK2_FBITS - fb) : 0u;
                rk[q] = atomicAdd(&tcnt[jj[q]], 1u);
                const uint32_t p = (uint32_t)((read_base + (uint64_t)(ga + lr[q]) * gsize) * M) + (rw[q] & 0xFFFFFFu);
#ifdef SK2_CHECK_P31
                assert((p >> 31) == 0);
#endif
                rw[q] = p | (uint32_t)sk2_canon(rx[q], ry[q], rz[q], k) << 31;
            }
        }
        __syncthreads();
        unsigned long long mybase = 0;
        unsigned int myv = 0;
        if (threadIdx.x < REFINE_FANOUT) {
            const unsigned int v = (int)threadIdx.x < F ? tcnt[threadIdx.x] : 0u;
            unsigned int incl = v;
            for (int o = 1; o < 64; o <<= 1) {
                const unsigned int u = __shfl_up(incl, o);
                if (lane >= o) incl += u;
            }
            tbeg[threadIdx.x] = incl - v;
            if (lane == 63) wsum[wid] = incl;
            myv = v;
            if (v) mybase = atomicAdd(&fcur[c * F + threadIdx.x], (unsigned long long)v);
        }
        __syncthreads();
        if (threadIdx.x >= 64 && threadIdx.x < REFINE_FANOUT) {
            unsigned int add = 0;
            for (int q = 0; q < (int)(threadIdx.x >> 6); q++) add += wsum[q];
            tbeg[threadIdx.x] += add;
        }
        __syncthreads();
#pragma unroll
        for (int q = 0; q < PER; q++) {
            const unsigned int i = threadIdx.x + q * BUCKET_THREADS;
            if (i < n) {
                const unsigned int p = tbeg[jj[q]] + rk[q];
                tile[p] = make_uint4(rx[q], ry[q], rz[q], rw[q]);
                tj[p] = (uint8_t)jj[q];
            }
        }
        if (threadIdx.x < REFINE_FANOUT) {
            if (mybase + myv > fcap) atomicOr(overflow, 1u);
            base[threadIdx.x] = (c * F + threadIdx.x) * fcap + mybase;
            tcnt[threadIdx.x] = mybase < fcap ? (unsigned int)min<unsigned long long>(fcap - mybase, 0xFFFFFFFFull) : 0u;
        }
        __syncthreads();
        for (unsigned int i = threadIdx.x; i < n; i += BUCKET_THREADS) {
            const unsigned int j = tj[i];
            const unsigned int q = i - tbeg[j];
            if (q < tcnt[j]) out[base[j] + q] = tile[i];
        }
        __syncthreads();
    }
}

template <int SLOTS>
struct LTabE {
    unsigned long long key[SLOTS];
    uint2 ev[SLOTS];
    unsigned int count[SLOTS];
};
struct EvExpand {
    unsigned int m2;
    __device__ inline unsigned long long one(unsigned int e) const {
        return ((unsigned long long)(e / m2) << 32) | (e % m2);
    }
    template <typename Tab>
    __device__ inline ulonglong2 operator()(const Tab &tab, int i) const {
        return make_ulonglong2(one(tab.ev[i].x), one(tab.ev[i].y));
    }
};


template <int SLOTS, int RS, int RB, bool EVEN_K>
__global__ void __launch_bounds__(BUCKET_THREADS) k_skbucket(const uint4 *recs, const unsigned long long *bbeg,
                                                             const unsigned long long *bend, int k, uint32_t M,
                                                             double inv_m, long long limit, unsigned long long *dkey,
                                                             unsigned int *dcnt, unsigned long long *dfc,
                                                             unsigned long long *dft, SubSlot *sub,
                                                             unsigned int *nsolid, unsigned long long *ndistinct,
                                                             unsigned int *overflow, unsigned long long *dbg) {
    constexpr int SBITS = SLOTS == 2048 ? 11 : 12;
    constexpr uint32_t PEND = 0x800u;
    constexpr unsigned int CLAIM_MAX = RS / 2 < RS - 1 - RB * BUCKET_THREADS ? RS / 2 : RS - 1 - RB * BUCKET_THREADS;
    static_assert(RS > RB * BUCKET_THREADS + 1, "record table too small for the records in flight");
    __shared__ LTabE<SLOTS> tab;
    __shared__ unsigned int s_over[2];
    __shared__ uint32_t r_tag[RS], r_x[RS], r_y[RS], r_z[RS], r_mult[RS], r_a[RS], r_b[RS];
    __shared__ uint16_t s_ord[RS];
    __shared__ unsigned int s_nent, s_ncnt[SK2_NMAX + 1];
    const unsigned int b = blockIdx.x, tid = threadIdx.x;
    for (int i = tid; i < SLOTS; i += BUCKET_THREADS) {
        tab.key[i] = EMPTY_KEY;
        tab.count[i] = 0;
        tab.ev[i] = make_uint2(0xFFFFFFFFu, 0xFFFFFFFFu);
    }
    for (int i = tid; i < RS; i += BUCKET_THREADS) {
        r_tag[i] = 0;
        r_mult[i] = 0;
        r_a[i] = r_b[i] = 0xFFFFFFFFu;
    }
    if (tid <= SK2_NMAX) s_ncnt[tid] = 0;
    if (tid == 0) s_over[0] = s_over[1] = 0, s_nent = 0;
    unsigned long long t_last = 0;
    auto phase = [&](int i) {
        if (dbg && tid == 0) {
            const unsigned long long t = wall_clock64();
            if (i) atomicAdd(&dbg[2 + i], t - t_last);
            t_last = t;
        }
    };
    phase(0);
    __syncthreads();
    const uint64_t r0 = bbeg[b], r1 = bend[b];
    const uint64_t kmask = kmask64(k);
    const int sh = 2 * (k - 1), fsh = 64 - 2 * k;

    unsigned long long n_rolled = 0;
    auto roll_out = [&](uint32_t x0, uint32_t x1, uint32_t x2, unsigned int mult, unsigned int ea, unsigned int eb) {
        const unsigned int n = (x2 >> 28) + 1;
        if (dbg) n_rolled += n;
        auto events = [&](uint64_t fwd, uint64_t rc, unsigned int o, unsigned int &eC, unsigned int &eT,
                          unsigned int &add) {
            const bool tw = fwd > rc;
            const unsigned int ef = ea + o, et = eb - o;
            add = mult;
            eC = tw ? et : ef;
            eT = tw ? ef : et;
            if (EVEN_K && fwd == rc) {
                add = 2 * mult;
                eC = eT = min(ef, et);
            }
            return tw ? rc : fwd;
        };
        const unsigned int h = (n + 1) >> 1;
        auto at = [&](unsigned int o, uint64_t &fw, uint64_t &rv) {
            const uint32_t lo = __builtin_amdgcn_alignbit(x1, x0, 2 * o), hi = __builtin_amdgcn_alignbit(x2, x1, 2 * o);
            const uint64_t P = (uint64_t)lo | (uint64_t)hi << 32;
            rv = ~P & kmask;
            fw = rev2_64(P) >> fsh;
        };
        auto roll = [&](unsigned int o, uint64_t &fw, uint64_t &rv) {
            const unsigned int tb = o + (unsigned int)k - 1;
            const uint32_t wd = tb < 32 ? x1 : x2;
            const uint32_t bb = (wd >> (2 * (tb & 15))) & 3u;
            fw = ((fw << 2) | bb) & kmask;
            rv = (rv >> 2) | ((uint64_t)(3u - bb) << sh);
        };
        uint64_t fA, rA, fB, rB;
        at(0, fA, rA);
        at(h, fB, rB);
        for (unsigned int i = 0; i < h; i++) {
            const unsigned int oB = i + h;
            const bool bB = oB < n;
            if (i) {
                roll(i, fA, rA);
                roll(oB, fB, rB);
            }
            unsigned int eCA, eTA, eCB, eTB, addA, addB;
            const uint64_t cA = events(fA, rA, i, eCA, eTA, addA);
            const uint64_t cB = events(fB, rB, oB, eCB, eTB, addB);
            unsigned int sA = (sk_slot(cA) >> (32 - SBITS)) & (SLOTS - 1), sB = (sk_slot(cB) >> (32 - SBITS)) & (SLOTS - 1);
            const unsigned long long kA = tab.key[sA], kB = tab.key[sB];
            lds_locate2<SLOTS>(tab, s_over, cA, sA, kA, cB, sB, bB ? kB : cB);
            atomicAdd(&tab.count[sA], addA);
            if (bB) atomicAdd(&tab.count[sB], addB);
            const uint2 vA = tab.ev[sA], vB = tab.ev[sB];
            if (eCA < vA.x) atomicMin(&tab.ev[sA].x, eCA);
            if (eTA < vA.y) atomicMin(&tab.ev[sA].y, eTA);
            if (bB && eCB < vB.x) atomicMin(&tab.ev[sB].x, eCB);
            if (bB && eTB < vB.y) atomicMin(&tab.ev[sB].y, eTB);
        }
    };

    constexpr unsigned int ROUND = RB * BUCKET_THREADS;
    phase(1);
    constexpr int PD = SK2_PD;
    uint4 nx[PD][RB];
#pragma unroll
    for (int d = 0; d < PD; d++)
#pragma unroll
        for (int j = 0; j < RB; j++) {
            const uint64_t ri = r0 + tid + (uint64_t)j * BUCKET_THREADS + (uint64_t)d * ROUND;
            nx[d][j] = recs[r1 > r0 ? min(ri, r1 - 1) : r0];
        }
    unsigned long long c_canon = 0, c_probe = 0, c_post = 0, n_iter = 0, n_rounds = 0, c_t = 0;
    auto tick = [&](unsigned long long &acc) {
        if (dbg) {
            const unsigned long long t = __builtin_amdgcn_s_memtime();
            acc += t - c_t;
            c_t = t;
        }
    };
    if (dbg) c_t = __builtin_amdgcn_s_memtime();
    auto record_round = [&](uint4 (&nxd)[RB], uint64_t c0) {
        if (dbg) n_rounds++;
        uint32_t K0[RB], K1[RB], K2[RB], EA[RB], EB[RB], TG[RB], SL[RB];
        int ST[RB];
#pragma unroll
        for (int j = 0; j < RB; j++) {
            const uint64_t ri = c0 + tid + (uint64_t)j * BUCKET_THREADS;
            const bool valid = ri < r1;
            const uint4 x = nxd[j];
            nxd[j] = recs[min(ri + PD * ROUND, r1 - 1)];
            const unsigned int n = (x.z >> 28) + 1;
            K0[j] = x.x, K1[j] = x.y, K2[j] = x.z;
            sk2_events(x.w, n, M, inv_m, EA[j], EB[j]);
            uint32_t hh = K0[j] * 0x9E3779B1u;
            hh = (hh ^ (hh >> 15) ^ K1[j]) * 0x85EBCA77u;
            hh = (hh ^ (hh >> 13) ^ K2[j]) * 0xC2B2AE3Du;
            hh ^= hh >> 16;
            TG[j] = (hh | 0x1000u) & 0xFFFFF000u;
            SL[j] = __umulhi(hh * 0x27D4EB2Fu, (unsigned int)RS);
            ST[j] = valid ? 0 : 1;
        }
        auto searching = [&]() {
            bool a = false;
#pragma unroll
            for (int j = 0; j < RB; j++) a |= ST[j] == 0;
            return a;
        };
        auto ld = [](uint32_t *a) { return __hip_atomic_load(a, __ATOMIC_RELAXED, __HIP_MEMORY_SCOPE_WORKGROUP); };
        tick(c_canon);
#pragma unroll 1
        while (__any(searching())) {
            if (dbg) n_iter++;
            uint32_t T[RB], X[RB], Y[RB], Z[RB];
#pragma unroll
            for (int j = 0; j < RB; j++) T[j] = ld(&r_tag[SL[j]]);
            asm volatile("" ::: "memory");
#pragma unroll
            for (int j = 0; j < RB; j++) X[j] = ld(&r_x[SL[j]]), Y[j] = ld(&r_y[SL[j]]), Z[j] = ld(&r_z[SL[j]]);
            bool claim = false;
#pragma unroll
            for (int j = 0; j < RB; j++) {
                const bool hit = T[j] == TG[j] && X[j] == K0[j] && Y[j] == K1[j] && Z[j] == K2[j];
                const bool go = ST[j] == 0;
                ST[j] = go && hit ? 1 : ST[j];
                claim |= go && !hit && T[j] == 0;
                if (go && !hit && T[j] != 0 && T[j] != (TG[j] | PEND))
                    SL[j] = SL[j] + 1 == (unsigned int)RS ? 0u : SL[j] + 1;
            }
            if (claim) {
#pragma unroll
                for (int j = 0; j < RB; j++) {
                    if (ST[j] != 0 || T[j] != 0) continue;
                    const unsigned int slot = SL[j];
                    if (ld(&s_nent) >= CLAIM_MAX) {
                        ST[j] = 2;
                    } else if (atomicCAS(&r_tag[slot], 0u, TG[j] | PEND) == 0) {
                        r_x[slot] = K0[j], r_y[slot] = K1[j], r_z[slot] = K2[j];
                        __hip_atomic_store(&r_tag[slot], TG[j], __ATOMIC_RELEASE, __HIP_MEMORY_SCOPE_WORKGROUP);
                        atomicAdd(&s_nent, 1u);
                        ST[j] = 1;
                    }
                }
            }
        }
        tick(c_probe);
#pragma unroll
        for (int j = 0; j < RB; j++) {
            const bool valid = c0 + tid + (uint64_t)j * BUCKET_THREADS < r1;
            if (valid && ST[j] == 1) {
                const unsigned int slot = SL[j];
                atomicAdd(&r_mult[slot], 1u);
                if (EA[j] < r_a[slot]) atomicMin(&r_a[slot], EA[j]);
                if (EB[j] < r_b[slot]) atomicMin(&r_b[slot], EB[j]);
            }
        }
#pragma unroll
        for (int j = 0; j < RB; j++)
            if (ST[j] == 2) roll_out(K0[j], K1[j], K2[j], 1u, EA[j], EB[j]);
        tick(c_post);
    };
    for (uint64_t c0 = r0; c0 < r1; c0 += PD * ROUND) {
#pragma unroll
        for (int d = 0; d < PD; d++) {
            if (c0 + (uint64_t)d * ROUND >= r1) break;
            record_round(nx[d], c0 + (uint64_t)d * ROUND);
        }
    }
    unsigned long long c_bar = 0;
    __syncthreads();
    tick(c_bar);
    if (dbg && (tid & 63) == 0) {
        atomicAdd(&dbg[8], c_canon), atomicAdd(&dbg[9], c_probe), atomicAdd(&dbg[10], c_post);
        atomicAdd(&dbg[11], n_iter), atomicAdd(&dbg[12], c_bar), atomicAdd(&dbg[13], n_rounds);
    }
    phase(2);
    {
        constexpr int PER = (RS + BUCKET_THREADS - 1) / BUCKET_THREADS;
        unsigned int sl[PER], rk[PER];
#pragma unroll
        for (int q = 0; q < PER; q++) {
            const unsigned int i = tid + q * BUCKET_THREADS;
            sl[q] = SK2_NMAX;
            if (i < (unsigned)RS && r_tag[i]) {
                sl[q] = SK2_NMAX - 1 - (r_z[i] >> 28);
                rk[q] = atomicAdd(&s_ncnt[sl[q]], 1u);
            }
        }
        __syncthreads();
        if (tid == 0) {
            unsigned int a = 0;
            for (int q = 0; q < SK2_NMAX; q++) {
                const unsigned int v = s_ncnt[q];
                s_ncnt[q] = a;
                a += v;
            }
            s_ncnt[SK2_NMAX] = a;
            if (dbg) atomicAdd(&dbg[0], (unsigned long long)a), atomicAdd(&dbg[1], 1ull);
        }
        __syncthreads();
#pragma unroll
        for (int q = 0; q < PER; q++)
            if (sl[q] < SK2_NMAX) s_ord[s_ncnt[sl[q]] + rk[q]] = (uint16_t)(tid + q * BUCKET_THREADS);
        __syncthreads();
        const unsigned int ne = s_ncnt[SK2_NMAX];
        phase(3);
        if (dbg) c_t = __builtin_amdgcn_s_memtime();
        unsigned long long c_roll = 0, c_bar2 = 0;
        for (unsigned int t = tid; t < ne; t += BUCKET_THREADS) {
            const unsigned int e = s_ord[t];
            roll_out(r_x[e], r_y[e], r_z[e], r_mult[e], r_a[e], r_b[e]);
        }
        tick(c_roll);
        __syncthreads();
        tick(c_bar2);
        if (dbg && (tid & 63) == 0) atomicAdd(&dbg[14], c_roll), atomicAdd(&dbg[15], c_bar2);
        if (dbg) atomicAdd(&dbg[2], n_rolled);
    }
    phase(4);
    lds_table_finish<SLOTS, false, KeyId>(tab, s_over, b, limit, dkey, dcnt, dfc, dft, sub, nsolid, ndistinct,
                                          overflow, KeyId(), EvExpand{2 * M});
    phase(5);
}


template <int SLOTS, int RS, int NT>
struct SkB3Lds {
    static constexpr int NC = RS / 2;
    struct Rec {
        uint32_t tag[RS], x[RS], y[RS], z[RS], mult[RS], a[RS], b[RS];
    };
    struct Roll {
        LTabE<SLOTS> tab;
        uint32_t x[NC], y[NC], z[NC], mult[NC], a[NC], b[NC];
    };
    union {
        Rec r;
        Roll k;
    };
};

template <int SLOTS, int RS, int NT, bool EVEN_K, bool STATS = false>
__global__ void __launch_bounds__(NT) k_skbucket3(const uint4 *recs, const unsigned long long *bbeg,
                                                  const unsigned long long *bend, int k, uint32_t M, double inv_m,
                                                  long long limit, unsigned long long *dkey, unsigned int *dcnt,
                                                  unsigned long long *dfc, unsigned long long *dft, SubSlot *sub,
                                                  unsigned int *nsolid, unsigned long long *ndistinct,
                                                  unsigned int *overflow, unsigned long long *dbg,
                                                  unsigned int claim_cap, unsigned int *bmark = nullptr) {
    constexpr int SBITS = __builtin_ctz(SLOTS);
    constexpr uint32_t PEND = 0x800u;
    constexpr unsigned int CLAIM_MAX = RS / 2 < RS - 1 - NT ? RS / 2 : RS - 1 - NT;
    static_assert(RS > NT + 1, "record table too small for the records in flight");
    static_assert(sizeof(typename SkB3Lds<SLOTS, RS, NT>::Roll) <= sizeof(typename SkB3Lds<SLOTS, RS, NT>::Rec),
                  "the k-mer table and the compact records fit the record table's space");
    constexpr int OV = 256;
    __shared__ SkB3Lds<SLOTS, RS, NT> L;
    __shared__ uint32_t o_x[OV], o_y[OV], o_z[OV], o_a[OV], o_b[OV];
    __shared__ unsigned int s_over[2];
    __shared__ unsigned int s_nent, s_nov, s_ncnt[SK2_NMAX + 1];
    auto &R = L.r;
    auto &tab = L.k.tab;
    const unsigned int b = blockIdx.x, tid = threadIdx.x;
    for (int i = tid; i < RS; i += NT) {
        R.tag[i] = 0;
        R.mult[i] = 0;
        R.a[i] = R.b[i] = 0xFFFFFFFFu;
    }
    if (tid <= SK2_NMAX) s_ncnt[tid] = 0;
    if (tid == 0) s_over[0] = s_over[1] = 0, s_nent = 0, s_nov = 0;
    __syncthreads();
    const uint64_t r0 = bbeg[b], r1 = bend[b];
    const uint64_t kmask = kmask64(k);
    const int sh = 2 * (k - 1), fsh = 64 - 2 * k;
    unsigned long long n_rolled = 0;

    auto roll_out = [&](uint32_t x0, uint32_t x1, uint32_t x2, unsigned int mult, unsigned int ea, unsigned int eb) {
        const unsigned int n = (x2 >> 28) + 1;
        if (dbg) n_rolled += n;
        auto events = [&](uint64_t fwd, uint64_t rc, unsigned int o, unsigned int &eC, unsigned int &eT,
                          unsigned int &add) {
            const bool tw = fwd > rc;
            const unsigned int ef = ea + o, et = eb - o;
            add = mult;
            eC = tw ? et : ef;
            eT = tw ? ef : et;
            if (EVEN_K && fwd == rc) {
                add = 2 * mult;
                eC = eT = min(ef, et);
            }
            return tw ? rc : fwd;
        };
        const unsigned int h = (n + 1) >> 1;
        auto at = [&](unsigned int o, uint64_t &fw, uint64_t &rv) {
            const uint32_t lo = __builtin_amdgcn_alignbit(x1, x0, 2 * o), hi = __builtin_amdgcn_alignbit(x2, x1, 2 * o);
            const uint64_t P = (uint64_t)lo | (uint64_t)hi << 32;
            rv = ~P & kmask;
            fw = rev2_64(P) >> fsh;
        };
        auto roll = [&](unsigned int o, uint64_t &fw, uint64_t &rv) {
            const unsigned int tb = o + (unsigned int)k - 1;
            const uint32_t wd = tb < 32 ? x1 : x2;
            const uint32_t bb = (wd >> (2 * (tb & 15))) & 3u;
            fw = ((fw << 2) | bb) & kmask;
            rv = (rv >> 2) | ((uint64_t)(3u - bb) << sh);
        };
        uint64_t fA, rA, fB, rB;
        at(0, fA, rA);
        at(h, fB, rB);
        for (unsigned int i = 0; i < h; i++) {
            const unsigned int oB = i + h;
            const bool bB = oB < n;
            if (i) {
                roll(i, fA, rA);
                roll(oB, fB, rB);
            }
            unsigned int eCA, eTA, eCB, eTB, addA, addB;
            const uint64_t cA = events(fA, rA, i, eCA, eTA, addA);
            const uint64_t cB = events(fB, rB, oB, eCB, eTB, addB);
            unsigned int sA = (sk_slot(cA) >> (32 - SBITS)) & (SLOTS - 1), sB = (sk_slot(cB) >> (32 - SBITS)) & (SLOTS - 1);
            const unsigned long long kA = tab.key[sA], kB = tab.key[sB];
            lds_locate2<SLOTS>(tab, s_over, cA, sA, kA, cB, sB, bB ? kB : cB);
            atomicAdd(&tab.count[sA], addA);
            if (bB) atomicAdd(&tab.count[sB], addB);
            const uint2 vA = tab.ev[sA], vB = tab.ev[sB];
            if (eCA < vA.x) atomicMin(&tab.ev[sA].x, eCA);
            if (eTA < vA.y) atomicMin(&tab.ev[sA].y, eTA);
            if (bB && eCB < vB.x) atomicMin(&tab.ev[sB].x, eCB);
            if (bB && eTB < vB.y) atomicMin(&tab.ev[sB].y, eTB);
        }
    };

    constexpr int PD = SK2_PD;
    uint4 nx[PD];
#pragma unroll
    for (int d = 0; d < PD; d++) nx[d] = recs[r1 > r0 ? min(r0 + tid + (uint64_t)d * NT, r1 - 1) : r0];
    auto ld = [](uint32_t *a) { return __hip_atomic_load(a, __ATOMIC_RELAXED, __HIP_MEMORY_SCOPE_WORKGROUP); };
    unsigned long long c_canon = 0, c_probe = 0, c_post = 0, n_iter = 0, n_rounds = 0, c_t = 0;
    auto tick = [&](unsigned long long &acc) {
        if constexpr (STATS) {
            const unsigned long long t = __builtin_amdgcn_s_memtime();
            acc += t - c_t;
            c_t = t;
        }
    };
    if constexpr (STATS) c_t = __builtin_amdgcn_s_memtime();
    auto record_round = [&](uint4 &nxd, uint64_t c0) {
        if constexpr (STATS) n_rounds++;
        const uint64_t ri = c0 + tid;
        const bool valid = ri < r1;
        const uint4 x = nxd;
        nxd = recs[min(ri + PD * NT, r1 - 1)];
        const unsigned int n = (x.z >> 28) + 1;
        const uint32_t K0 = x.x, K1 = x.y, K2 = x.z;
        uint32_t EA, EB;
        sk2_events(x.w, n, M, inv_m, EA, EB);
        uint32_t hh = K0 * 0x9E3779B1u;
        hh = (hh ^ (hh >> 15) ^ K1) * 0x85EBCA77u;
        hh = (hh ^ (hh >> 13) ^ K2) * 0xC2B2AE3Du;
        hh ^= hh >> 16;
        const uint32_t TG = (hh | 0x1000u) & 0xFFFFF000u;
        uint32_t SL = __umulhi(hh * 0x27D4EB2Fu, (unsigned int)RS);
        int ST = valid ? 0 : 1;
        tick(c_canon);
#pragma unroll 1
        while (__any(ST == 0)) {
            if constexpr (STATS) n_iter++;
            const uint32_t T = ld(&R.tag[SL]);
            asm volatile("" ::: "memory");
            const uint32_t X = ld(&R.x[SL]), Y = ld(&R.y[SL]), Z = ld(&R.z[SL]);
            const bool hit = T == TG && X == K0 && Y == K1 && Z == K2;
            const bool go = ST == 0;
            ST = go && hit ? 1 : ST;
            const bool claim = go && !hit && T == 0;
            if (go && !hit && T != 0 && T != (TG | PEND)) SL = SL + 1 == (unsigned int)RS ? 0u : SL + 1;
            if (claim) {
                const unsigned int o = atomicAdd(&s_nent, 1u);
                if (o >= min(CLAIM_MAX, claim_cap)) {
                    atomicSub(&s_nent, 1u);
                    ST = 2;
                } else if (atomicCAS(&R.tag[SL], 0u, TG | PEND) == 0) {
                    R.x[SL] = K0, R.y[SL] = K1, R.z[SL] = K2;
                    __hip_atomic_store(&R.tag[SL], TG, __ATOMIC_RELEASE, __HIP_MEMORY_SCOPE_WORKGROUP);
                    ST = 1;
                } else {
                    atomicSub(&s_nent, 1u);
                }
            }
        }
        tick(c_probe);
        if (valid && ST == 1) {
            atomicAdd(&R.mult[SL], 1u);
            if (EA < R.a[SL]) atomicMin(&R.a[SL], EA);
            if (EB < R.b[SL]) atomicMin(&R.b[SL], EB);
        }
        if (ST == 2) {
            const unsigned int o = atomicAdd(&s_nov, 1u);
            if (o < (unsigned int)OV) o_x[o] = K0, o_y[o] = K1, o_z[o] = K2, o_a[o] = EA, o_b[o] = EB;
            else s_over[0] = 1;
        }
        tick(c_post);
    };
    for (uint64_t c0 = r0; c0 < r1; c0 += PD * NT) {
#pragma unroll
        for (int d = 0; d < PD; d++) {
            if (c0 + (uint64_t)d * NT >= r1) break;
            record_round(nx[d], c0 + (uint64_t)d * NT);
        }
    }
    __syncthreads();
    if constexpr (STATS) {
        unsigned long long c_bar = 0;
        tick(c_bar);
        if ((tid & 63) == 0) {
            atomicAdd(&dbg[8], c_canon), atomicAdd(&dbg[9], c_probe), atomicAdd(&dbg[10], c_post);
            atomicAdd(&dbg[11], n_iter), atomicAdd(&dbg[12], c_bar), atomicAdd(&dbg[13], n_rounds);
        }
    }
    constexpr int PER = (RS + NT - 1) / NT;
    uint32_t cx[PER], cy[PER], cz[PER], cm[PER], ca[PER], cb[PER], bin[PER], rk[PER];
#pragma unroll
    for (int q = 0; q < PER; q++) {
        const unsigned int i = tid + q * NT;
        bin[q] = SK2_NMAX;
        if (i < (unsigned)RS && R.tag[i]) {
            cx[q] = R.x[i], cy[q] = R.y[i], cz[q] = R.z[i], cm[q] = R.mult[i], ca[q] = R.a[i], cb[q] = R.b[i];
            bin[q] = SK2_NMAX - 1 - (cz[q] >> 28);
            rk[q] = atomicAdd(&s_ncnt[bin[q]], 1u);
        }
    }
    __syncthreads();
    if (tid == 0) {
        unsigned int a = 0;
        for (int q = 0; q < SK2_NMAX; q++) {
            const unsigned int v = s_ncnt[q];
            s_ncnt[q] = a;
            a += v;
        }
        s_ncnt[SK2_NMAX] = a;
        if (dbg) {
            atomicAdd(&dbg[0], (unsigned long long)a), atomicAdd(&dbg[1], 1ull);
            atomicMax(&dbg[3], (unsigned long long)(a + min(s_nov, (unsigned int)OV)));
        }
    }
    for (int i = tid; i < SLOTS; i += NT) {
        tab.key[i] = EMPTY_KEY;
        tab.count[i] = 0;
        tab.ev[i] = make_uint2(0xFFFFFFFFu, 0xFFFFFFFFu);
    }
    __syncthreads();
#pragma unroll
    for (int q = 0; q < PER; q++)
        if (bin[q] < SK2_NMAX) {
            const unsigned int o = s_ncnt[bin[q]] + rk[q];
            L.k.x[o] = cx[q], L.k.y[o] = cy[q], L.k.z[o] = cz[q], L.k.mult[o] = cm[q], L.k.a[o] = ca[q], L.k.b[o] = cb[q];
        }
    __syncthreads();
    const unsigned int ne = s_ncnt[SK2_NMAX], nov = min(s_nov, (unsigned int)OV);
    if constexpr (STATS) c_t = __builtin_amdgcn_s_memtime();
    for (unsigned int t = tid; t < ne + nov; t += NT) {
        if (t < ne) roll_out(L.k.x[t], L.k.y[t], L.k.z[t], L.k.mult[t], L.k.a[t], L.k.b[t]);
        else {
            const unsigned int o = t - ne;
            roll_out(o_x[o], o_y[o], o_z[o], 1u, o_a[o], o_b[o]);
        }
    }
    if constexpr (STATS) {
        unsigned long long c_roll = 0, c_bar2 = 0;
        tick(c_roll);
        __syncthreads();
        tick(c_bar2);
        if ((tid & 63) == 0) atomicAdd(&dbg[14], c_roll), atomicAdd(&dbg[15], c_bar2);
    }
    if (dbg) atomicAdd(&dbg[2], n_rolled);
    lds_table_finish<SLOTS, false, KeyId, LTabE<SLOTS>, EvExpand, NT>(tab, s_over, b, limit, dkey, dcnt, dfc, dft, sub,
                                                                      nsolid, ndistinct, overflow, KeyId(),
                                                                      EvExpand{2 * M}, bmark);
}


constexpr int SKF_BITS = 17;
template <int SLOTS, int NT, bool EVEN_K, bool MERGED = false>
__global__ void __launch_bounds__(NT) k_skbucket_filt(const uint4 *recs, const unsigned long long *bbeg,
                                                      const unsigned long long *bend, int k, uint32_t M, double inv_m,
                                                      long long limit, unsigned long long *dkey, unsigned int *dcnt,
                                                      unsigned long long *dfc, unsigned long long *dft, SubSlot *sub,
                                                      unsigned int *nsolid, unsigned long long *ndistinct,
                                                      unsigned int *overflow, unsigned int max_keys,
                                                      unsigned long long *dbg = nullptr, unsigned int *bmark = nullptr,
                                                      const uint2 *mev = nullptr) {
    constexpr int SBITS = __builtin_ctz(SLOTS);
    constexpr unsigned int NW = 1u << (SKF_BITS - 5), CM = (1u << SKF_BITS) - 1;
    __shared__ LTabE<SLOTS> tab;
    __shared__ unsigned int s_over[2];
    __shared__ unsigned int seen1[NW], seen2[NW];
    __shared__ unsigned int s_cells[2];
    const unsigned int b = blockIdx.x, tid = threadIdx.x;
    for (int i = tid; i < SLOTS; i += NT) {
        tab.key[i] = EMPTY_KEY;
        tab.count[i] = 0;
        tab.ev[i] = make_uint2(0xFFFFFFFFu, 0xFFFFFFFFu);
    }
    for (unsigned int i = tid; i < NW; i += NT) seen1[i] = seen2[i] = 0;
    if (tid == 0) s_over[0] = s_over[1] = 0, s_cells[0] = s_cells[1] = 0;
    __syncthreads();
    const uint64_t r0 = bbeg[b], r1 = bend[b];
    const uint64_t kmask = kmask64(k);
    const int fsh = 64 - 2 * k;
    auto windows = [&](uint64_t ri, const uint4 &x, auto &&fn) {
        const unsigned int n = (x.z >> 28) + 1;
        uint32_t EA, EB;
        unsigned int mult = 1;
        if constexpr (MERGED) {
            const uint2 e = mev[ri];
            EA = e.x, EB = e.y, mult = x.w;
        } else {
            sk2_events(x.w, n, M, inv_m, EA, EB);
        }
        for (unsigned int o = 0; o < n; o++) {
            const uint32_t lo = __builtin_amdgcn_alignbit(x.y, x.x, 2 * o), hi = __builtin_amdgcn_alignbit(x.z, x.y, 2 * o);
            const uint64_t P = (uint64_t)lo | (uint64_t)hi << 32;
            const uint64_t rv = ~P & kmask, fw = rev2_64(P) >> fsh;
            const bool tw = fw > rv;
            const unsigned int ef = EA + o, et = EB - o;
            unsigned int add = mult, eC = tw ? et : ef, eT = tw ? ef : et;
            if (EVEN_K && fw == rv) {
                add = 2 * mult;
                eC = eT = min(ef, et);
            }
            fn(tw ? rv : fw, add, eC, eT);
        }
    };
    auto cells = [](unsigned long long c, unsigned int &c1, unsigned int &c2) {
        const uint64_t h = mix64(c);
        c1 = (unsigned int)(h >> 12) & CM;
        c2 = (unsigned int)(h >> 30) & CM;
    };
    for (uint64_t i = r0 + tid; i < r1; i += NT) {
        const uint4 x = recs[i];
        const bool rep = MERGED && x.w > 1;
        windows(i, x, [&](unsigned long long c, unsigned int, unsigned int, unsigned int) {
            unsigned int c1, c2;
            cells(c, c1, c2);
            const unsigned int m1 = 1u << (c1 & 31), mm2 = 1u << (c2 & 31);
            if (rep) {
                atomicOr(&seen1[c1 >> 5], m1), atomicOr(&seen2[c1 >> 5], m1);
                atomicOr(&seen1[c2 >> 5], mm2), atomicOr(&seen2[c2 >> 5], mm2);
                return;
            }
            if (atomicOr(&seen1[c1 >> 5], m1) & m1) atomicOr(&seen2[c1 >> 5], m1);
            if (atomicOr(&seen1[c2 >> 5], mm2) & mm2) atomicOr(&seen2[c2 >> 5], mm2);
        });
    }
    __syncthreads();
    {
        unsigned int n2 = 0, n1 = 0;
        for (unsigned int i = tid; i < NW; i += NT) n2 += __popc(seen2[i]), n1 += __popc(seen1[i]);
        for (int o = 32; o > 0; o >>= 1) n2 += __shfl_down(n2, o), n1 += __shfl_down(n1, o);
        if ((tid & 63) == 0) atomicAdd(&s_cells[0], n2), atomicAdd(&s_cells[1], n1);
        __syncthreads();
        if (tid == 0) {
            const double m = (double)(1u << SKF_BITS);
            const double D = -m * log(1.0 - (double)min(s_cells[1], CM) / m) / 2.0;
            const double l = 2.0 * D / m, el = exp(-l);
            const double S = fmax(0.0, ((double)s_cells[0] - m * (1.0 - el * (1.0 + l))) / 2.0);
            const double pass = 1.1 * (S + fmax(0.0, D - S) * (1.0 - el) * (1.0 - el));
            if (pass > (double)max_keys) s_over[0] = 1;
            else atomicAdd(ndistinct, (unsigned long long)llround(D));
            if (dbg) {
                atomicMax(&dbg[0], (unsigned long long)D);
                atomicMax(&dbg[1], (unsigned long long)pass);
                atomicMax(&dbg[2], (unsigned long long)s_cells[0]);
                atomicMax(&dbg[3], (unsigned long long)(bend[b] - bbeg[b]));
                if (s_over[0]) atomicAdd(&dbg[4], 1ull);
            }
        }
        __syncthreads();
    }
    if (s_over[0]) {
        if (tid == 0) atomicAdd(overflow, 1u);
        return;
    }
    for (uint64_t i = r0 + tid; i < r1; i += NT) {
        windows(i, recs[i], [&](unsigned long long c, unsigned int add, unsigned int eC, unsigned int eT) {
            if ((long long)add <= limit) {
                unsigned int c1, c2;
                cells(c, c1, c2);
                const bool twice = ((seen2[c1 >> 5] >> (c1 & 31)) & (seen2[c2 >> 5] >> (c2 & 31)) & 1u) != 0;
                if (!twice) return;
            }
            const unsigned int s0 = (sk_slot(c) >> (32 - SBITS)) & (SLOTS - 1);
            const unsigned int sl = lds_locate<SLOTS>(tab, s_over, c, s0, tab.key[s0]);
            atomicAdd(&tab.count[sl], add);
            const uint2 v = tab.ev[sl];
            if (eC < v.x) atomicMin(&tab.ev[sl].x, eC);
            if (eT < v.y) atomicMin(&tab.ev[sl].y, eT);
        });
    }
    if (dbg) {
        __syncthreads();
        if (tid == 0) {
            if (s_over[0]) atomicAdd(&dbg[5], 1ull);
            atomicMax(&dbg[6], (unsigned long long)s_over[1]);
        }
    }
    lds_table_finish<SLOTS, false, KeyId, LTabE<SLOTS>, EvExpand, NT>(tab, s_over, b, limit, dkey, dcnt, dfc, dft, sub,
                                                                      nsolid, nullptr, overflow, KeyId(),
                                                                      EvExpand{2 * M}, bmark);
}


template <int RS, int NT>
__global__ void __launch_bounds__(NT) k_skdedup(const uint4 *recs, const unsigned long long *bbeg,
                                                const unsigned long long *bend, int k, uint32_t M, double inv_m,
                                                uint4 *mrec, uint2 *mev, unsigned long long *mend,
                                                unsigned int claim_cap = ~0u, unsigned long long *dbg = nullptr) {
    constexpr uint32_t PEND = 0x800u;
    constexpr unsigned int CLAIM_MAX = RS - 1 - NT;
    static_assert(RS > NT + 1, "record table too small for the records in flight");
    __shared__ uint32_t tag[RS], tx[RS], ty[RS], tz[RS], tm[RS], ta[RS], tb[RS];
    __shared__ unsigned int s_nent, s_nout, s_nrej, s_ncnt[SK2_NMAX];
    const unsigned int b = blockIdx.x, tid = threadIdx.x;
    for (int i = tid; i < RS; i += NT) {
        tag[i] = 0;
        tm[i] = 0;
        ta[i] = tb[i] = 0xFFFFFFFFu;
    }
    if (tid == 0) s_nent = 0, s_nout = 0, s_nrej = 0;
    if (tid < (unsigned int)SK2_NMAX) s_ncnt[tid] = 0;
    __syncthreads();
    const uint64_t r0 = bbeg[b], r1 = bend[b];
    auto ld = [](uint32_t *a) { return __hip_atomic_load(a, __ATOMIC_RELAXED, __HIP_MEMORY_SCOPE_WORKGROUP); };
    uint4 nxt = r1 > r0 ? recs[min(r0 + tid, r1 - 1)] : make_uint4(0u, 0u, 0u, 0u);
    for (uint64_t c0 = r0; c0 < r1; c0 += NT) {
        const uint64_t ri = c0 + tid;
        const bool valid = ri < r1;
        const uint4 x = nxt;
        if (c0 + NT < r1) nxt = recs[min(ri + NT, r1 - 1)];
        const unsigned int n = (x.z >> 28) + 1;
        const uint32_t K0 = x.x, K1 = x.y, K2 = x.z;
        uint32_t EA, EB;
        sk2_events(x.w, n, M, inv_m, EA, EB);
        uint32_t hh = K0 * 0x9E3779B1u;
        hh = (hh ^ (hh >> 15) ^ K1) * 0x85EBCA77u;
        hh = (hh ^ (hh >> 13) ^ K2) * 0xC2B2AE3Du;
        hh ^= hh >> 16;
        const uint32_t TG = (hh | 0x1000u) & 0xFFFFF000u;
        uint32_t SL = __umulhi(hh * 0x27D4EB2Fu, (unsigned int)RS);
        int ST = valid ? 0 : 1;
#pragma unroll 1
        while (__any(ST == 0)) {
            const uint32_t T = ld(&tag[SL]);
            asm volatile("" ::: "memory");
            const uint32_t X = ld(&tx[SL]), Y = ld(&ty[SL]), Z = ld(&tz[SL]);
            const bool hit = T == TG && X == K0 && Y == K1 && Z == K2;
            const bool go = ST == 0;
            ST = go && hit ? 1 : ST;
            const bool claim = go && !hit && T == 0;
            if (go && !hit && T != 0 && T != (TG | PEND)) SL = SL + 1 == (unsigned int)RS ? 0u : SL + 1;
            if (claim) {
                const unsigned int o = atomicAdd(&s_nent, 1u);
                if (o >= min(CLAIM_MAX, claim_cap)) {
                    atomicSub(&s_nent, 1u);
                    ST = 2;
                } else if (atomicCAS(&tag[SL], 0u, TG | PEND) == 0) {
                    tx[SL] = K0, ty[SL] = K1, tz[SL] = K2;
                    __hip_atomic_store(&tag[SL], TG, __ATOMIC_RELEASE, __HIP_MEMORY_SCOPE_WORKGROUP);
                    ST = 1;
                } else {
                    atomicSub(&s_nent, 1u);
                }
            }
        }
        if (valid && ST == 1) {
            atomicAdd(&tm[SL], 1u);
            if (EA < ta[SL]) atomicMin(&ta[SL], EA);
            if (EB < tb[SL]) atomicMin(&tb[SL], EB);
        }
        if (ST == 2) {
            if (dbg) atomicAdd(&s_nrej, 1u);
            const uint64_t o = r0 + atomicAdd(&s_nout, 1u);
            mrec[o] = make_uint4(K0, K1, K2, 1u);
            mev[o] = make_uint2(EA, EB);
        }
    }
    __syncthreads();
    constexpr int PER = (RS + NT - 1) / NT;
    uint32_t bin[PER], rk[PER];
#pragma unroll
    for (int q = 0; q < PER; q++) {
        const unsigned int i = tid + q * NT;
        bin[q] = SK2_NMAX;
        if (i < (unsigned int)RS && tag[i]) {
            bin[q] = SK2_NMAX - 1 - (tz[i] >> 28);
            rk[q] = atomicAdd(&s_ncnt[bin[q]], 1u);
        }
    }
    __syncthreads();
    if (tid == 0) {
        unsigned int a = s_nout;
        for (int q = 0; q < SK2_NMAX; q++) {
            const unsigned int v = s_ncnt[q];
            s_ncnt[q] = a;
            a += v;
        }
        s_nout = a;
    }
    __syncthreads();
#pragma unroll
    for (int q = 0; q < PER; q++) {
        if (bin[q] == SK2_NMAX) continue;
        const unsigned int i = tid + q * NT;
        const uint64_t o = r0 + s_ncnt[bin[q]] + rk[q];
        mrec[o] = make_uint4(tx[i], ty[i], tz[i], tm[i]);
        mev[o] = make_uint2(ta[i], tb[i]);
    }
    __syncthreads();
    if (tid == 0) {
        mend[b] = r0 + s_nout;
        if (dbg) {
            atomicMax(&dbg[7], (unsigned long long)s_nout);
            atomicMax(&dbg[8], (unsigned long long)s_nrej);
            atomicAdd(&dbg[9], (unsigned long long)s_nout);
        }
    }
}

}
```

Before: 197.9 billion.

## Encode super-k-mer event positions with power-of-two stride to avoid division

Adds a pow-2 event encoding in which each read gets a stride of 2^lgE rather than 2*M. Event A/B computation becomes an XOR with a mask, and expansion uses shifts and masks in place of double-precision divide and modulo in the bucket, dedup and filter kernels. The refine kernel now does the position and canonical-flip encoding up front. It falls back to the exact form when the larger stride would overflow the 32-bit or 24-bit limits, and an env flag forces the exact form.

```diff
diff --git a/pycuda-euler_amd/csrc/assemble.hip b/pycuda-euler_amd/csrc/assemble.hip
--- a/pycuda-euler_amd/csrc/assemble.hip
+++ b/pycuda-euler_amd/csrc/assemble.hip
@@ -176,6 +176,7 @@
         bool valid = false;
         uint64_t G = 0, cap = 0, nreads = 0, read_base = 0, fcap = 0;
         uint32_t M = 0;
+        uint32_t lgE = 0;
         int k = 0, bbits = 0;
     } skspec;
     struct JlSpec {
@@ -666,9 +667,12 @@
         gsize = ((ntiles + g - 1) / g) * 64;
         G = (nreads + gsize - 1) / gsize;
     }
-    if (k < SK_MIN_K || k > 32 || M > 256 || gsize * M >= (1ull << 24) || (read_base + nreads) * 2 * M >= (1ull << 32) ||
-        kn().no_sk2)
-        return EC_OK;
+    uint32_t lgE = 0;
+    const Sk2Form form = sk2_event_form(M, nreads, read_base, gsize, kn().sk2_exact, &lgE);
+    if (k < SK_MIN_K || k > 32 || form == SK2_FORM_NONE || kn().no_sk2) return EC_OK;
+    const uint32_t pstride = lgE ? 1u << (lgE - 1) : M;
+    if (kn().verbose || kn().sk2_stats)
+        fprintf(stderr, "count_sk2: events in the %s form (stride %u)\n", lgE ? "pow-2" : "exact", lgE ? 1u << lgE : 2 * M);
     hipStream_t st = s->stream;
     Scalars *dsc = s->scal.as<Scalars>();
     Scalars hsc;
@@ -701,7 +705,7 @@
 #define EC_SKPART_WV(NPF, W, VAL)                                                                             \
     k_skpart_w<NPF, W, VAL><<<lgb - lga, PT_THREADS, 0, st>>>(                                                   \
         d_reads, d_off, nreads, mc, M, gsize, (uint32_t)G, cap, smask, recs, s->cnt.as<unsigned int>(),          \
-        s->hll.as<uint8_t>(), &dsc->nrec, &dsc->overflow, &dsc->lens[2], &dsc->npos, lga, elim)
+        s->hll.as<uint8_t>(), &dsc->nrec, &dsc->overflow, &dsc->lens[2], &dsc->npos, lga, elim, pstride)
 #define EC_SKPART_W(NPF, W)            \
     if (validate)                      \
         EC_SKPART_WV(NPF, W, true);    \
@@ -762,7 +766,7 @@
         k_skrefine<<<dim3((unsigned)C, rs), BUCKET_THREADS, 0, st>>>(recs, s->cnt.as<unsigned int>(), (uint32_t)G, cap,
                                                                       bb, s->recs2.as<uint4>(), fc,
                                                                       s->fcur.as<unsigned long long>(), &dsc->skew, M,
-                                                                      gsize, read_base, k);
+                                                                      gsize, read_base, k, lgE);
         kmark(s, 4, 1);
         unsigned long long *b0 = s->bb2.as<unsigned long long>();
         k_fixed_bounds<<<grid_for(nb, 256), 256, 0, st>>>(s->fcur.as<unsigned long long>(), nb, fc, b0, b0 + nb);
@@ -770,7 +774,7 @@
     };
     const auto sp = s->skspec;
     const bool spec = sp.valid && sp.G == G && sp.cap == cap && sp.nreads == nreads && sp.read_base == read_base &&
-                      sp.M == M && sp.k == k && !chunked && kn().no_spec == 0;
+                      sp.M == M && sp.k == k && sp.lgE == lgE && !chunked && kn().no_spec == 0;
     s->skspec.valid = false;
     if (spec) {
         if (!s->rd_ev) EC_HIP(hipEventCreateWithFlags(&s->rd_ev, hipEventDisableTiming));
@@ -825,6 +829,7 @@
     s->skspec.M = M;
     s->skspec.k = k;
     s->skspec.bbits = bbits;
+    s->skspec.lgE = lgE;
     unsigned long long *bbeg = s->bb2.as<unsigned long long>(), *bend = bbeg + Bk;
     mark(s, 2 * EC_STAGE_COUNT + 1);
 
@@ -840,7 +845,7 @@
     kmark(s, 2, 0);
     const double inv_m = 1.0 / M;
 #define EC_SKBUCKET_ARGS                                                                                     \
-    s->recs2.as<uint4>(), bbeg, bend, k, M, inv_m, limit, s->dkey.as<unsigned long long>(),                    \
+    s->recs2.as<uint4>(), bbeg, bend, k, M, inv_m, lgE, limit, s->dkey.as<unsigned long long>(),               \
         s->dcnt.as<unsigned int>(), s->dfc.as<unsigned long long>(), s->dft.as<unsigned long long>(),          \
         s->no_index ? nullptr : s->sub.as<SubSlot>(), &dsc->nsolid, &dsc->ndistinct, &dsc->overflow
 #define EC_SKBUCKET(SLOTS, RS, EVEN) \
@@ -865,13 +870,13 @@
             unsigned long long *mend = s->skm_end.as<unsigned long long>();
             const unsigned int claim_cap = kn().sk2_claim > 0 ? (unsigned int)kn().sk2_claim : ~0u;
             if (kn().skf_merge != 2)
-                k_skdedup<4096, 1024><<<(unsigned)Bk, 1024, 0, st>>>(s->recs2.as<uint4>(), bbeg, bend, k, M, inv_m, mrec,
+                k_skdedup<4096, 1024><<<(unsigned)Bk, 1024, 0, st>>>(s->recs2.as<uint4>(), bbeg, bend, k, M, inv_m, lgE, mrec,
                                                                      mev, mend, claim_cap, dbg);
             else
-                k_skdedup<2560, 512><<<(unsigned)Bk, 512, 0, st>>>(s->recs2.as<uint4>(), bbeg, bend, k, M, inv_m, mrec,
+                k_skdedup<2560, 512><<<(unsigned)Bk, 512, 0, st>>>(s->recs2.as<uint4>(), bbeg, bend, k, M, inv_m, lgE, mrec,
                                                                    mev, mend, claim_cap, dbg);
 #define EC_SKF_MERGED_ARGS                                                                                   \
-    mrec, bbeg, mend, k, M, inv_m, limit, s->dkey.as<unsigned long long>(), s->dcnt.as<unsigned int>(),      \
+    mrec, bbeg, mend, k, M, inv_m, lgE, limit, s->dkey.as<unsigned long long>(), s->dcnt.as<unsigned int>(), \
         s->dfc.as<unsigned long long>(), s->dft.as<unsigned long long>(),                                    \
         s->no_index ? nullptr : s->sub.as<SubSlot>(), &dsc->nsolid, &dsc->ndistinct, &dsc->overflow, max_keys, \
         dbg, bm, mev
diff --git a/pycuda-euler_amd/csrc/capi.cpp b/pycuda-euler_amd/csrc/capi.cpp
--- a/pycuda-euler_amd/csrc/capi.cpp
+++ b/pycuda-euler_amd/csrc/capi.cpp
@@ -46,6 +46,7 @@
         k.junction_claim = num("EULERHIP_JUNCTION_CLAIM", 0);
         if (const char *e = getenv("EULERHIP_WIDE_L3_CAP")) k.wide_l3_cap = atoll(e);
         k.host_chunks = num("EULERHIP_HOST_CHUNKS", 0);
+        k.sk2_exact = flag("EULERHIP_SK2_EXACT");
         k.sk2_stats = flag("EULERHIP_SK2_STATS");
         k.no_skb3 = flag("EULERHIP_NO_SKB3");
         k.sk2_claim = num("EULERHIP_SK2_CLAIM", 0);
diff --git a/pycuda-euler_amd/csrc/common.h b/pycuda-euler_amd/csrc/common.h
--- a/pycuda-euler_amd/csrc/common.h
+++ b/pycuda-euler_amd/csrc/common.h
@@ -43,6 +43,7 @@
     int no_char_pack = 0;
     int sk2_elim = 0;
     int sk2_claim = 0;
+    bool sk2_exact = false;
     bool sk2_stats = false;
     bool no_skb3 = false;
     int sk_filt = -1;
diff --git a/pycuda-euler_amd/csrc/count_sk2.h b/pycuda-euler_amd/csrc/count_sk2.h
--- a/pycuda-euler_amd/csrc/count_sk2.h
+++ b/pycuda-euler_amd/csrc/count_sk2.h
@@ -1,5 +1,6 @@
 #pragma once
 #include "count_v2.h"
+#include "sk2_form.h"
 #include "superkmer.h"
 
 namespace ec {
@@ -45,9 +46,10 @@
 __device__ inline void skpart_flush(uint32_t cntw, const uint32_t *ent, uint16_t *srt, unsigned int *wcnt,
                                     unsigned int *cur, unsigned long long *base, const uint32_t *rel,
                                     const uint32_t *st, uint32_t lane, unsigned long long gcap, uint64_t cap,
-                                    unsigned long long spill, uint32_t M, uint32_t rtile, uint4 *recs,
+                                    unsigned long long spill, uint32_t pstride, uint32_t rtile, uint4 *recs,
                                     unsigned int *overflow, unsigned int *s_hll, uint32_t *hq, uint32_t smaskb,
                                     int k, uint64_t kmask) {
+    const uint32_t pbase = rtile * pstride;
     wave_sync();
     for (uint32_t i = lane; i < cntw; i += 64) atomicAdd(&wcnt[ent[i] >> 26], 1u);
     wave_sync();
@@ -98,7 +100,7 @@
             o.x = sk_bases16(st, p0);
             o.y = sk_bases16(st, p0 + 16);
             o.z = (sk_bases16(st, p0 + 32) & 0x0FFFFFFFu) | n1 << 28;
-            o.w = ((e >> 18) & ((1u << SK2_FBITS) - 1)) << 24 | ((rtile + lr) * M + w0);
+            o.w = ((e >> 18) & ((1u << SK2_FBITS) - 1)) << 24 | (pbase + __umul24(lr, pstride) + w0);
             recs[base[e >> 26] + i] = o;
             samp = ((e >> 18) & smaskb) == 0;
             qv = p0 | n1 << 16;
@@ -120,7 +122,7 @@
                                                          uint32_t smask, uint4 *recs, unsigned int *cnt, uint8_t *hll,
                                                          unsigned long long *nrec, unsigned int *overflow,
                                                          unsigned int *vfail, unsigned long long *npos,
-                                                         uint32_t g_lo, uint32_t elim) {
+                                                         uint32_t g_lo, uint32_t elim, uint32_t pstride) {
     constexpr int C = 1 << SK2_CBITS;
     constexpr int NREG = 1 << HLL_REG_BITS;
     constexpr int SW = NPF * 64 + 4;
@@ -279,7 +281,7 @@
             }
             if (round + 1 < nrounds && cntw > elim - 64 - 640) {
                 skpart_flush<C>(cntw, ent, s_srt[wid], s_wcnt[wid], s_cur, s_base[wid], s_rel[wid], st, lane, gcap,
-                                cap, spill, M, rtile, recs, overflow, s_hll, s_hq[wid], smask ? 0xFFu : 0u, k,
+                                cap, spill, pstride, rtile, recs, overflow, s_hll, s_hq[wid], smask ? 0xFFu : 0u, k,
                                 kmask);
                 cntw = 0;
             }
@@ -294,7 +296,7 @@
             }
             cntw += (uint32_t)__popcll(bal);
             skpart_flush<C>(cntw, ent, s_srt[wid], s_wcnt[wid], s_cur, s_base[wid], s_rel[wid], st, lane, gcap,
-                            cap, spill, M, rtile, recs, overflow, s_hll, s_hq[wid], smask ? 0xFFu : 0u, k, kmask);
+                            cap, spill, pstride, rtile, recs, overflow, s_hll, s_hq[wid], smask ? 0xFFu : 0u, k, kmask);
         }
     }
     __shared__ unsigned int s_nwin[PT_WAVES];
@@ -334,7 +336,12 @@
     r0 = flip ? q0 : x0, r1 = flip ? q1 : x1, r2 = (flip ? q2 : x2) | (n - 1) << 28;
     return flip;
 }
-__device__ inline void sk2_events(uint32_t w, unsigned int n, uint32_t M, double inv_m, uint32_t &EA, uint32_t &EB) {
+__device__ inline void sk2_events(uint32_t w, unsigned int n, uint32_t M, double inv_m, uint32_t emask, uint32_t &EA,
+                                  uint32_t &EB) {
+    if (emask) {
+        EA = w, EB = w ^ emask;
+        return;
+    }
     const unsigned int p = w & 0x7FFFFFFFu;
     const bool flip = (w >> 31) != 0;
     const unsigned int rd0 = (unsigned int)((double)p * inv_m);
@@ -346,10 +353,21 @@
     EA = flip ? B - n + 1 : A, EB = flip ? A + n - 1 : B;
 }
 
+template <int RS>
+__device__ inline void sk2_rec_hash(uint32_t K0, uint32_t K1, uint32_t K2, uint32_t &TG, uint32_t &SL) {
+    uint32_t hh = K0 * 0x9E3779B1u;
+    hh = (hh ^ (hh >> 15) ^ K1) * 0x85EBCA77u;
+    hh = (hh ^ (hh >> 13) ^ K2) * 0xC2B2AE3Du;
+    hh ^= hh >> 16;
+    TG = (hh | 0x1000u) & 0xFFFFF000u;
+    SL = __umulhi(hh * 0x27D4EB2Fu, (unsigned int)RS);
+}
+
 __global__ void __launch_bounds__(BUCKET_THREADS) k_skrefine(const uint4 *recs, const unsigned int *cnt, uint32_t G,
                                                              uint64_t cap, int bbits, uint4 *out, uint64_t fcap,
                                                              unsigned long long *fcur, unsigned int *overflow,
-                                                             uint32_t M, uint64_t gsize, uint64_t read_base, int k) {
+                                                             uint32_t M, uint64_t gsize, uint64_t read_base, int k,
+                                                             uint32_t lgE) {
     constexpr int TILE = SK2_TILE;
     constexpr int PER = TILE / BUCKET_THREADS;
     constexpr uint64_t C = 1 << SK2_CBITS;
@@ -408,11 +426,23 @@
             if (i < n) {
                 jj[q] = fb ? (rw[q] >> 24) >> (SK2_FBITS - fb) : 0u;
                 rk[q] = atomicAdd(&tcnt[jj[q]], 1u);
-                const uint32_t p = (uint32_t)((read_base + (uint64_t)(ga + lr[q]) * gsize) * M) + (rw[q] & 0xFFFFFFu);
-#ifdef SK2_CHECK_P31
-                assert((p >> 31) == 0);
+                const uint32_t rdg = (uint32_t)read_base + __umul24(ga + lr[q], (uint32_t)gsize);
+                const uint32_t rel = rw[q] & 0xFFFFFFu;
+                const bool flip = sk2_canon(rx[q], ry[q], rz[q], k);
+                if (lgE) {
+                    const uint32_t w0 = rel & ((1u << (lgE - 1)) - 1u), hi = rel - w0;
+#ifdef SK2_CHECK_EV
+                    assert((((uint64_t)rdg + (rel >> (lgE - 1)) + 1) << lgE) <= (1ull << 32));
 #endif
-                rw[q] = p | (uint32_t)sk2_canon(rx[q], ry[q], rz[q], k) << 31;
+                    const uint32_t e0 = flip ? (1u << lgE) - 1u - (rz[q] >> 28) - w0 : w0;
+                    rw[q] = (hi << 1) + ((rdg << lgE) + e0);
+                } else {
+                    const uint32_t p = rdg * M + rel;
+#ifdef SK2_CHECK_EV
+                    assert(((uint64_t)rdg * M + rel) >> 31 == 0);
+#endif
+                    rw[q] = p | (uint32_t)flip << 31;
+                }
             }
         }
         __syncthreads();
@@ -469,7 +499,12 @@
 };
 struct EvExpand {
     unsigned int m2;
+    unsigned int lgE;
     __device__ inline unsigned long long one(unsigned int e) const {
+        if (lgE) {
+            const unsigned int E = 1u << lgE, lp = e & (E - 1);
+            return ((unsigned long long)(e >> lgE) << 32) | (lp < (E >> 1) ? lp : lp - (E - m2));
+        }
         return ((unsigned long long)(e / m2) << 32) | (e % m2);
     }
     template <typename Tab>
@@ -482,7 +517,8 @@
 template <int SLOTS, int RS, int RB, bool EVEN_K>
 __global__ void __launch_bounds__(BUCKET_THREADS) k_skbucket(const uint4 *recs, const unsigned long long *bbeg,
                                                              const unsigned long long *bend, int k, uint32_t M,
-                                                             double inv_m, long long limit, unsigned long long *dkey,
+                                                             double inv_m, uint32_t lgE, long long limit,
+                                                             unsigned long long *dkey,
                                                              unsigned int *dcnt, unsigned long long *dfc,
                                                              unsigned long long *dft, SubSlot *sub,
                                                              unsigned int *nsolid, unsigned long long *ndistinct,
@@ -521,6 +557,7 @@
     __syncthreads();
     const uint64_t r0 = bbeg[b], r1 = bend[b];
     const uint64_t kmask = kmask64(k);
+    const uint32_t emask = lgE ? (1u << lgE) - 1u : 0u;
     const int sh = 2 * (k - 1), fsh = 64 - 2 * k;
 
     unsigned long long n_rolled = 0;
@@ -612,13 +649,8 @@
             nxd[j] = recs[min(ri + PD * ROUND, r1 - 1)];
             const unsigned int n = (x.z >> 28) + 1;
             K0[j] = x.x, K1[j] = x.y, K2[j] = x.z;
-            sk2_events(x.w, n, M, inv_m, EA[j], EB[j]);
-            uint32_t hh = K0[j] * 0x9E3779B1u;
-            hh = (hh ^ (hh >> 15) ^ K1[j]) * 0x85EBCA77u;
-            hh = (hh ^ (hh >> 13) ^ K2[j]) * 0xC2B2AE3Du;
-            hh ^= hh >> 16;
-            TG[j] = (hh | 0x1000u) & 0xFFFFF000u;
-            SL[j] = __umulhi(hh * 0x27D4EB2Fu, (unsigned int)RS);
+            sk2_events(x.w, n, M, inv_m, emask, EA[j], EB[j]);
+            sk2_rec_hash<RS>(K0[j], K1[j], K2[j], TG[j], SL[j]);
             ST[j] = valid ? 0 : 1;
         }
         auto searching = [&]() {
@@ -739,7 +771,7 @@
     }
     phase(4);
     lds_table_finish<SLOTS, false, KeyId>(tab, s_over, b, limit, dkey, dcnt, dfc, dft, sub, nsolid, ndistinct,
-                                          overflow, KeyId(), EvExpand{2 * M});
+                                          overflow, KeyId(), EvExpand{2 * M, lgE});
     phase(5);
 }
 
@@ -763,7 +795,7 @@
 template <int SLOTS, int RS, int NT, bool EVEN_K, bool STATS = false>
 __global__ void __launch_bounds__(NT) k_skbucket3(const uint4 *recs, const unsigned long long *bbeg,
                                                   const unsigned long long *bend, int k, uint32_t M, double inv_m,
-                                                  long long limit, unsigned long long *dkey, unsigned int *dcnt,
+                                                  uint32_t lgE, long long limit, unsigned long long *dkey, unsigned int *dcnt,
                                                   unsigned long long *dfc, unsigned long long *dft, SubSlot *sub,
                                                   unsigned int *nsolid, unsigned long long *ndistinct,
                                                   unsigned int *overflow, unsigned long long *dbg,
@@ -792,6 +824,7 @@
     __syncthreads();
     const uint64_t r0 = bbeg[b], r1 = bend[b];
     const uint64_t kmask = kmask64(k);
+    const uint32_t emask = lgE ? (1u << lgE) - 1u : 0u;
     const int sh = 2 * (k - 1), fsh = 64 - 2 * k;
     unsigned long long n_rolled = 0;
 
@@ -874,13 +907,9 @@
         const unsigned int n = (x.z >> 28) + 1;
         const uint32_t K0 = x.x, K1 = x.y, K2 = x.z;
         uint32_t EA, EB;
-        sk2_events(x.w, n, M, inv_m, EA, EB);
-        uint32_t hh = K0 * 0x9E3779B1u;
-        hh = (hh ^ (hh >> 15) ^ K1) * 0x85EBCA77u;
-        hh = (hh ^ (hh >> 13) ^ K2) * 0xC2B2AE3Du;
-        hh ^= hh >> 16;
-        const uint32_t TG = (hh | 0x1000u) & 0xFFFFF000u;
-        uint32_t SL = __umulhi(hh * 0x27D4EB2Fu, (unsigned int)RS);
+        sk2_events(x.w, n, M, inv_m, emask, EA, EB);
+        uint32_t TG, SL;
+        sk2_rec_hash<RS>(K0, K1, K2, TG, SL);
         int ST = valid ? 0 : 1;
         tick(c_canon);
 #pragma unroll 1
@@ -995,7 +1024,7 @@
     if (dbg) atomicAdd(&dbg[2], n_rolled);
     lds_table_finish<SLOTS, false, KeyId, LTabE<SLOTS>, EvExpand, NT>(tab, s_over, b, limit, dkey, dcnt, dfc, dft, sub,
                                                                       nsolid, ndistinct, overflow, KeyId(),
-                                                                      EvExpand{2 * M}, bmark);
+                                                                      EvExpand{2 * M, lgE}, bmark);
 }
 
 
@@ -1003,7 +1032,7 @@
 template <int SLOTS, int NT, bool EVEN_K, bool MERGED = false>
 __global__ void __launch_bounds__(NT) k_skbucket_filt(const uint4 *recs, const unsigned long long *bbeg,
                                                       const unsigned long long *bend, int k, uint32_t M, double inv_m,
-                                                      long long limit, unsigned long long *dkey, unsigned int *dcnt,
+                                                      uint32_t lgE, long long limit, unsigned long long *dkey, unsigned int *dcnt,
                                                       unsigned long long *dfc, unsigned long long *dft, SubSlot *sub,
                                                       unsigned int *nsolid, unsigned long long *ndistinct,
                                                       unsigned int *overflow, unsigned int max_keys,
@@ -1026,6 +1055,7 @@
     __syncthreads();
     const uint64_t r0 = bbeg[b], r1 = bend[b];
     const uint64_t kmask = kmask64(k);
+    const uint32_t emask = lgE ? (1u << lgE) - 1u : 0u;
     const int fsh = 64 - 2 * k;
     auto windows = [&](uint64_t ri, const uint4 &x, auto &&fn) {
         const unsigned int n = (x.z >> 28) + 1;
@@ -1035,7 +1065,7 @@
             const uint2 e = mev[ri];
             EA = e.x, EB = e.y, mult = x.w;
         } else {
-            sk2_events(x.w, n, M, inv_m, EA, EB);
+            sk2_events(x.w, n, M, inv_m, emask, EA, EB);
         }
         for (unsigned int o = 0; o < n; o++) {
             const uint32_t lo = __builtin_amdgcn_alignbit(x.y, x.x, 2 * o), hi = __builtin_amdgcn_alignbit(x.z, x.y, 2 * o);
@@ -1126,14 +1156,14 @@
     }
     lds_table_finish<SLOTS, false, KeyId, LTabE<SLOTS>, EvExpand, NT>(tab, s_over, b, limit, dkey, dcnt, dfc, dft, sub,
                                                                       nsolid, nullptr, overflow, KeyId(),
-                                                                      EvExpand{2 * M}, bmark);
+                                                                      EvExpand{2 * M, lgE}, bmark);
 }
 
 
 template <int RS, int NT>
 __global__ void __launch_bounds__(NT) k_skdedup(const uint4 *recs, const unsigned long long *bbeg,
                                                 const unsigned long long *bend, int k, uint32_t M, double inv_m,
-                                                uint4 *mrec, uint2 *mev, unsigned long long *mend,
+                                                uint32_t lgE, uint4 *mrec, uint2 *mev, unsigned long long *mend,
                                                 unsigned int claim_cap = ~0u, unsigned long long *dbg = nullptr) {
     constexpr uint32_t PEND = 0x800u;
     constexpr unsigned int CLAIM_MAX = RS - 1 - NT;
@@ -1150,6 +1180,7 @@
     if (tid < (unsigned int)SK2_NMAX) s_ncnt[tid] = 0;
     __syncthreads();
     const uint64_t r0 = bbeg[b], r1 = bend[b];
+    const uint32_t emask = lgE ? (1u << lgE) - 1u : 0u;
     auto ld = [](uint32_t *a) { return __hip_atomic_load(a, __ATOMIC_RELAXED, __HIP_MEMORY_SCOPE_WORKGROUP); };
     uint4 nxt = r1 > r0 ? recs[min(r0 + tid, r1 - 1)] : make_uint4(0u, 0u, 0u, 0u);
     for (uint64_t c0 = r0; c0 < r1; c0 += NT) {
@@ -1160,13 +1191,9 @@
         const unsigned int n = (x.z >> 28) + 1;
         const uint32_t K0 = x.x, K1 = x.y, K2 = x.z;
         uint32_t EA, EB;
-        sk2_events(x.w, n, M, inv_m, EA, EB);
-        uint32_t hh = K0 * 0x9E3779B1u;
-        hh = (hh ^ (hh >> 15) ^ K1) * 0x85EBCA77u;
-        hh = (hh ^ (hh >> 13) ^ K2) * 0xC2B2AE3Du;
-        hh ^= hh >> 16;
-        const uint32_t TG = (hh | 0x1000u) & 0xFFFFF000u;
-        uint32_t SL = __umulhi(hh * 0x27D4EB2Fu, (unsigned int)RS);
+        sk2_events(x.w, n, M, inv_m, emask, EA, EB);
+        uint32_t TG, SL;
+        sk2_rec_hash<RS>(K0, K1, K2, TG, SL);
         int ST = valid ? 0 : 1;
 #pragma unroll 1
         while (__any(ST == 0)) {
diff --git a/pycuda-euler_amd/csrc/sk2_form.h b/pycuda-euler_amd/csrc/sk2_form.h
--- /dev/null
+++ b/pycuda-euler_amd/csrc/sk2_form.h
@@ -0,0 +1,22 @@
+#pragma once
+#include <stdint.h>
+
+namespace ec {
+
+enum Sk2Form { SK2_FORM_NONE = 0, SK2_FORM_EXACT = 1, SK2_FORM_POW2 = 2 };
+
+inline Sk2Form sk2_event_form(uint32_t M, uint64_t nreads, uint64_t read_base, uint64_t gsize, bool force_exact,
+                              uint32_t *lgE) {
+    if (lgE) *lgE = 0;
+    if (M < 1 || M > 256 || gsize * M >= (1ull << 24) || (read_base + nreads) * 2 * M >= (1ull << 32))
+        return SK2_FORM_NONE;
+    uint32_t lg = 1;
+    while ((1u << lg) < 2 * M) lg++;
+    const uint64_t E = 1ull << lg;
+    if (force_exact || (read_base + nreads) * E >= (1ull << 32) || gsize * (E / 2) >= (1ull << 24))
+        return SK2_FORM_EXACT;
+    if (lgE) *lgE = lg;
+    return SK2_FORM_POW2;
+}
+
+}
```

Result: no change. 199.2 billion (median of 4 runs) (+0.6%).
